# ryought/dbgphmm

Hardware: AMD Instinct MI355X
Metric: read-bases/sec through forward+backward P(R|X) (higher is better)
Workload: dtype f64

## Files before the change

dbgphmm_amd/csrc/api.cpp:

```cpp
#include <chrono>
#include <cstdlib>
#include <cmath>
#include <cstring>

#include "phmm_internal.h"

namespace phmm {

static thread_local std::string g_error;
static thread_local hipStream_t g_stream = nullptr;
static thread_local uint64_t g_ws_limit = 0;
static thread_local CallStats g_stats;
static thread_local bool g_timing = false;

void set_error(const std::string &msg) { g_error = msg; }
int fail(int code, const std::string &msg) {
    g_error = msg;
    return code;
}
hipStream_t current_stream() { return g_stream; }
int &workset_index() {
    static thread_local int idx = 0;
    return idx;
}
ThreadContext capture_thread_context() {
    ThreadContext c{g_ws_limit, g_timing, 0};
    (void)hipGetDevice(&c.device);
    return c;
}
void adopt_thread_context(const ThreadContext &c, hipStream_t stream, int workset) {
    (void)hipSetDevice(c.device);
    g_ws_limit = c.ws_limit;
    g_timing = c.timing;
    g_stream = stream;
    g_stats = CallStats();
    workset_index() = workset;
}
CallStats &stats() { return g_stats; }
bool timing_enabled() { return g_timing; }

uint64_t workspace_limit() {
    if (g_ws_limit) return g_ws_limit;
    size_t fr = 0, tot = 0;
    if (hipMemGetInfo(&fr, &tot) != hipSuccess) return (uint64_t)16 << 30;
    return (uint64_t)(0.8 * (double)fr);
}

static Knobs g_knobs;
const Knobs &knobs() { return g_knobs; }
void refresh_knobs() {
    auto flag = [](const char *n) {
        const char *e = std::getenv(n);
        return e != nullptr && e[0] != '\0' && !(e[0] == '0' && e[1] == '\0');
    };
    auto num = [](const char *n, int dflt) {
        const char *e = std::getenv(n);
        return e ? std::atoi(e) : dflt;
    };
    Knobs k;
    k.trace = flag("PHMM_TRACE");
    k.no_lean = flag("PHMM_NO_LEAN");
    k.no_wide_class = flag("PHMM_NO_WIDE_CLASS");
    k.no_packed = flag("PHMM_NO_PACKED");
    k.packed_cpl = num("PHMM_PACKED_CPL", 0);
    k.no_exact_hinted = flag("PHMM_NO_EXACT_HINTED");
    k.no_exact_dense = flag("PHMM_NO_EXACT_DENSE");
    k.no_wide_hinted = flag("PHMM_NO_WIDE_HINTED");
    k.wide_hinted = flag("PHMM_WIDE_HINTED") && !k.no_wide_hinted;
    k.wide_hinted_cpb = num("PHMM_WIDE_HINTED_CPB", 0);
    if (k.wide_hinted_cpb != 1 && k.wide_hinted_cpb != 2 && k.wide_hinted_cpb != 4) k.wide_hinted_cpb = 0;
    k.no_side_worker = flag("PHMM_NO_SIDE_WORKER");
    k.no_wide_handover = flag("PHMM_NO_WIDE_HANDOVER");
    k.workers = std::max(1, std::min(MAX_WORKERS, num("PHMM_WORKERS", 1)));
    k.warm_cols = num("PHMM_WARM_COLS", 0);
    k.chunk_groups = std::max(0, num("PHMM_CHUNK_GROUPS", 0));
    k.no_keep_all = flag("PHMM_NO_KEEP_ALL");
    k.pipeline_min_groups = std::max(1, num("PHMM_PIPELINE_MIN_GROUPS", 8));
    k.no_runmax = flag("PHMM_NO_RUNMAX");
    k.force_radix = flag("PHMM_FORCE_RADIX");
    k.no_bwd_skip = flag("PHMM_NO_BWD_SKIP");
    k.serial_emit = flag("PHMM_SERIAL_EMIT");
    k.emit_high_priority = flag("PHMM_EMIT_HIGH_PRIORITY");
    k.no_dma = flag("PHMM_NO_DMA");
    k.bwd_dma = flag("PHMM_BWD_DMA");
    k.dense_streams = num("PHMM_DENSE_STREAMS", 0);
    k.dense_w = num("PHMM_DENSE_W", 0);
    k.dense_npt = num("PHMM_DENSE_NPT", 0);
    if (const char *e = std::getenv("PHMM_MEM_FRACTION")) k.mem_fraction = std::min(0.97, std::max(0.1, std::atof(e)));
    g_knobs = k;
}

void trace(const char *tag) {
    if (!g_knobs.trace) return;
    static thread_local std::chrono::steady_clock::time_point last = std::chrono::steady_clock::now();
    (void)hipStreamSynchronize(g_stream);
    const auto now = std::chrono::steady_clock::now();
    static const auto t0 = std::chrono::steady_clock::now();
    std::fprintf(stderr, "[phmm trace] w%d @%9.2f %-28s %8.2f ms\n", workset_index(),
                 std::chrono::duration<double, std::milli>(now - t0).count(), tag,
                 std::chrono::duration<double, std::milli>(now - last).count());
    last = now;
}

uint64_t table_budget(const DevicePool &pool, uint64_t reserve) {
    if (g_ws_limit) return g_ws_limit;
    size_t fr = 0, tot = 0;
    if (hipMemGetInfo(&fr, &tot) != hipSuccess) return (uint64_t)16 << 30;
    const double frac = g_knobs.mem_fraction > 0.0 ? g_knobs.mem_fraction : 0.9;
    const double b = frac * (double)(fr + pool.owned_table_bytes()) - (double)reserve;
    return (uint64_t)std::max(b, 64.0 * 1024 * 1024);
}
uint64_t planned_budget(const DevicePool &pool) {
    if (g_ws_limit) return g_ws_limit;
    size_t fr = 0, tot = 0;
    if (hipMemGetInfo(&fr, &tot) != hipSuccess) return (uint64_t)16 << 30;
    const double frac = g_knobs.mem_fraction > 0.0 ? g_knobs.mem_fraction : 0.95;
    return (uint64_t)(frac * (double)(fr + pool.owned_bytes()));
}

static std::mutex g_pool_mu;
static DevicePool *g_pools[64] = {};
DevicePool &device_pool() {
    int dev = 0;
    (void)hipGetDevice(&dev);
    if (dev < 0 || dev >= 64) PHMM_THROW(PHMM_ENODEVICE, "device index out of range");
    std::lock_guard<std::mutex> lk(g_pool_mu);
    if (!g_pools[dev]) {
        g_pools[dev] = new DevicePool();
        g_pools[dev]->device = dev;
    }
    return *g_pools[dev];
}
void DevicePool::recycle(DevBuf &b) {
    if (!b.p) return;
    std::lock_guard<std::mutex> lk(spare_mu);
    if (b.bytes < ((size_t)1 << 20) || b.bytes > SPARE_BYTES) {
        b.release();
        return;
    }
    while (!spare.empty() && (spare.size() >= SPARE_MAX || spare_total + b.bytes > SPARE_BYTES)) {
        (void)hipFree(spare.front().first);
        spare_total -= spare.front().second;
        spare.erase(spare.begin());
    }
    spare_total += b.bytes;
    const size_t n = b.bytes;
    spare.emplace_back(b.detach(), n);
}
void DevicePool::take(DevBuf &b, size_t n) {
    if (n <= b.bytes) return;
    {
        std::lock_guard<std::mutex> lk(spare_mu);
        int best = -1;
        for (int i = 0; i < (int)spare.size(); i++)
            if (spare[i].second >= n && spare[i].second <= 2 * n &&
                (best < 0 || spare[i].second < spare[best].second))
                best = i;
        if (best >= 0) {
            b.adopt(spare[best].first, spare[best].second);
            spare_total -= spare[best].second;
            spare.erase(spare.begin() + best);
            return;
        }
    }
    b.reserve(n);
}
void DevicePool::flush_spares() {
    std::lock_guard<std::mutex> lk(spare_mu);
    for (auto &e : spare) (void)hipFree(e.first);
    spare.clear();
    spare_total = 0;
}
void flush_spare_buffers() { device_pool().flush_spares(); }

void DevicePool::release() {
    flush_spares();
    for (auto &w : wsets) w.release();
    ws_out.release();
    for (auto &ws : wstream)
        if (ws) {
            (void)hipStreamDestroy(ws);
            ws = nullptr;
        }
    for (auto &ws : cstream)
        if (ws) {
            (void)hipStreamDestroy(ws);
            ws = nullptr;
        }
    for (auto &we : cevent)
        for (auto &e : we)
            if (e) {
                (void)hipEventDestroy(e);
                e = nullptr;
            }
}

void copy_out(void *dst, const void *src_dev, size_t bytes) {
    if (!dst || !bytes) return;
    hipPointerAttribute_t at;
    const bool dev = hipPointerGetAttributes(&at, dst) == hipSuccess && at.type == hipMemoryTypeDevice;
    if (!dev) (void)hipGetLastError();
    HIP_CHECK(hipMemcpyAsync(dst, src_dev, bytes, dev ? hipMemcpyDeviceToDevice : hipMemcpyDeviceToHost,
                             current_stream()));
    HIP_CHECK(hipStreamSynchronize(current_stream()));
}

void put_bytes(void *dst, const void *src, size_t n) {
    if (!dst || !n) return;
    hipPointerAttribute_t at;
    if (hipPointerGetAttributes(&at, dst) == hipSuccess && at.type == hipMemoryTypeDevice) {
        HIP_CHECK(hipMemcpyAsync(dst, src, n, hipMemcpyHostToDevice, current_stream()));
        HIP_CHECK(hipStreamSynchronize(current_stream()));
    } else {
        (void)hipGetLastError();
        std::memcpy(dst, src, n);
    }
}
void put_doubles(double *dst, const double *src, size_t n) { put_bytes(dst, src, n * sizeof(double)); }

void mappings_materialize_host(const phmm_mappings *cmp) {
    if (cmp->host_valid) return;
    auto *mp = const_cast<phmm_mappings *>(cmp);
    mp->pos_off.resize(mp->total_pos + 1);
    mp->nodes.resize(mp->total_entries);
    mp->logp.resize(mp->total_entries);
    HIP_CHECK(hipMemcpy(mp->pos_off.data(), mp->d_pos_off.p, sizeof(uint64_t) * (mp->total_pos + 1), hipMemcpyDeviceToHost));
    if (mp->total_entries) {
        HIP_CHECK(hipMemcpy(mp->nodes.data(), mp->d_nodes.p, sizeof(uint32_t) * mp->total_entries, hipMemcpyDeviceToHost));
        HIP_CHECK(hipMemcpy(mp->logp.data(), mp->d_logp.p, sizeof(double) * mp->total_entries, hipMemcpyDeviceToHost));
    }
    mp->host_valid = true;
}

// ... 758 lines not shown
```

dbgphmm_amd/csrc/dense.hip:

```cpp
#include <algorithm>
#include <cmath>
#include <cstring>
#include <numeric>
#include <type_traits>

#include "dense_internal.h"
#include "lds_dma.h"

#ifndef PHMM_FWD_PF
#define PHMM_FWD_PF 2
#endif
#ifndef PHMM_BWD_PF
#define PHMM_BWD_PF 1
#endif
#ifndef PHMM_SMALLW_WAVES
#define PHMM_SMALLW_WAVES 3
#endif

namespace phmm {


__device__ __forceinline__ int xcd_block(int b, int nblk8) {
    int per = nblk8 >> 3;
    return (b & 7) * per + (b >> 3);
}

__device__ __forceinline__ NodeRec load_node(const NodeRec *nodes, int k) {
    typedef const NodeRec __attribute__((address_space(4))) *KPtr;
    const KPtr q = (KPtr)(uintptr_t)nodes;
    NodeRec r;
    r.init = q[k].init;
    r.dinit = q[k].dinit;
    r.tdinit = q[k].tdinit;
    r.emis = q[k].emis;
    r.flags = q[k].flags;
    return r;
}

__device__ __forceinline__ void wait_vmcnt(int n) {
#define PHMM_VMW(k) case k: asm volatile("s_waitcnt vmcnt(" #k ")" ::: "memory"); break;
    switch (n) {
        PHMM_VMW(1) PHMM_VMW(2) PHMM_VMW(3) PHMM_VMW(4) PHMM_VMW(5) PHMM_VMW(6) PHMM_VMW(7) PHMM_VMW(8)
        PHMM_VMW(9) PHMM_VMW(10) PHMM_VMW(11) PHMM_VMW(12) PHMM_VMW(13) PHMM_VMW(14) PHMM_VMW(15) PHMM_VMW(16)
        PHMM_VMW(17) PHMM_VMW(18) PHMM_VMW(19) PHMM_VMW(20) PHMM_VMW(21) PHMM_VMW(22) PHMM_VMW(23) PHMM_VMW(24)
        PHMM_VMW(25) PHMM_VMW(26) PHMM_VMW(27) PHMM_VMW(28) PHMM_VMW(29) PHMM_VMW(30) PHMM_VMW(31)
    default: asm volatile("s_waitcnt vmcnt(0)" ::: "memory"); break;
    }
#undef PHMM_VMW
}
#ifndef PHMM_DMA_DEPTH
#define PHMM_DMA_DEPTH 4
#endif
static constexpr int DMA_DEPTH = PHMM_DMA_DEPTH;
static_assert(DMA_DEPTH - 1 + DMA_DEPTH * 3 <= 31, "vmcnt immediates");

__device__ __forceinline__ int exp_of_bits(unsigned long long bits) {
    int be = (int)((bits >> 52) & 0x7ff);
    if (bits == 0ull) return 0;
    if (be == 0) return -1022;
    return be - 1022;
}
__device__ __forceinline__ double pow2(int e) {
    return __longlong_as_double((long long)(e + 1023) << 52);
}

template <int W, class Op>
__device__ __forceinline__ double block_reduce_rows(double v, Op op, double *lds) {
#pragma unroll
    for (int off = W; off < 64; off <<= 1) v = op(v, __shfl_xor(v, off));
    const int wave = threadIdx.x >> 6, lane = threadIdx.x & 63;
    __syncthreads();
    if (lane < W) lds[wave * 64 + lane] = v;
    __syncthreads();
    double out = v;
    if (threadIdx.x < W) {
        out = lds[threadIdx.x];
#pragma unroll
        for (int w = 1; w < BLOCK / 64; w++) out = op(out, lds[w * 64 + threadIdx.x]);
    }
    return out;
}
template <int W> __device__ __forceinline__ double lanes_sum(double v) {
    if (W == 16) {
        auto ror = [](double x, auto ctrl) {
            const long long b = __double_as_longlong(x);
            const int lo = __builtin_amdgcn_update_dpp(0, (int)(b & 0xffffffffll), decltype(ctrl)::value, 0xf, 0xf, false);
            const int hi = __builtin_amdgcn_update_dpp(0, (int)(b >> 32), decltype(ctrl)::value, 0xf, 0xf, false);
            return __longlong_as_double(((long long)hi << 32) | (long long)(unsigned int)lo);
        };
        v += ror(v, std::integral_constant<int, 0x128>());
        v += ror(v, std::integral_constant<int, 0x124>());
        v += ror(v, std::integral_constant<int, 0x122>());
        v += ror(v, std::integral_constant<int, 0x121>());
        return v;
    }
#pragma unroll
    for (int off = 1; off < W; off <<= 1) v += __shfl_xor(v, off);
    return v;
}

struct OpMax {
    __device__ double operator()(double a, double b) const { return a > b ? a : b; }
};
struct OpAdd {
    __device__ double operator()(double a, double b) const { return a + b; }
};

template <int W, bool DMA>
__global__ void __launch_bounds__(BLOCK, (W == 64 ? 4 : PHMM_SMALLW_WAVES)) fwd_step(const DenseArgs a, const int pos) {
    __shared__ double lds[(BLOCK / 64) * 64];
    constexpr bool DMA_ = DMA && W == 64;
    __shared__ double ring[DMA_ ? (BLOCK / 64) * DMA_DEPTH * 128 : 1];
    const int g = blockIdx.y + a.g_off;
    const int lb = xcd_block(blockIdx.x, a.nblk8);
    constexpr int ROWS = BLOCK / W;
    const int r = threadIdx.x % W;
    const int row = threadIdx.x / W;
    const int len = a.len[g * W + r];
    const bool active = a.wf_sw == nullptr || a.wf_sw[g * W + r] < 0;
    const bool newcol = active && pos < len;
    const bool have_prev = active && pos >= 1 && pos <= len;
    const bool fin = have_prev && pos == len;
    if (!__syncthreads_or(newcol || have_prev)) return;
    const LinParams &lp = a.lp;
    const size_t NW = (size_t)a.N * W;

    int Epos = 0;
    double sc = 1.0, isc = 1.0, ibs = 0.0;
    double thrL = INFINITY, thrU = INFINITY;
    bool collect = false;
    if (have_prev) {
        const unsigned long long cm = a.cmaxF[((size_t)g * a.Lc + (pos - 1)) * W + r];
        const int Eprev = a.FE[((size_t)g * (a.Lc + 1) + (pos - 1)) * W + r];
        const double ib_st = exp(a.logib[pos - 1] - (double)Eprev * LN2);
        const unsigned long long ibb = (unsigned long long)__double_as_longlong(ib_st);
        const int e = exp_of_bits(cm > ibb ? cm : ibb);
        sc = pow2(-e);
        isc = pow2(e);
        Epos = Eprev + e;
        ibs = exp(a.logib[pos - 1] - (double)Epos * LN2);
        if (a.wf_sw) {
            const double cmF = __longlong_as_double((long long)cm) * sc;
            thrL = cmF * a.wf_ratio;
            thrU = (a.wf_ub_a * cmF + a.wf_ub_b * lp.p_ID * ibs) * (1.0 + 1e-9) * a.wf_ratio;
            collect = a.wf_mode[g * W + r] != 0;
        }
    }
    const uint8_t x = newcol ? a.bases[((size_t)g * a.Lc + pos) * W + r] : (uint8_t)0;

    const double *pm = a.Fm + ((size_t)g * a.Lc + (pos > 0 ? pos - 1 : 0)) * NW;
    const double *pi = a.Fi + ((size_t)g * a.Lc + (pos > 0 ? pos - 1 : 0)) * NW;
    double *pd = a.Fd + ((size_t)g * a.Lc + (pos > 0 ? pos - 1 : 0)) * NW;
// ... 101 lines not shown
                        D4 = wg[0] + q * (wg[1] + q * (wg[2] + q * wg[3]));
                        D5 = wg[0] + q * (wg[1] + q * (wg[2] + q * (wg[3] + q * wg[4])));
                        Tk = 0.0;
#pragma unroll
                        for (int h = H - 1; h >= 1; h--)
                            if (h <= lp.n_max_gaps + 1) Tk = wg[h] + q * Tk;
                        nvalid = 1;
                    }
                    m1 = wm0;
                    i1 = wi0;
                    const int G = lp.n_max_gaps;
                    dacc = G == 4 ? D5 : (G == 3 ? D4 : (G == 2 ? D3 : (G == 1 ? D2 : D1)));
                    tacc = Tk;
                } else {
                    m1 = i1 = dacc = tacc = 0.0;
                    const uint32_t o0 = a.fc_off[k], o1 = a.fc_off[k + 1];
                    for (uint32_t q = o0; q < o1; q++) {
                        const FwdEntry en = a.fc[q];
                        const size_t ix = (size_t)en.node * W + r;
                        const double vm = pm[ix] * sc, vi = pi[ix] * sc;
                        const double gg = lp.p_MD * vm + lp.p_ID * vi;
                        m1 += en.w1 * vm;
                        i1 += en.w1 * vi;
                        dacc += en.wD * gg;
                        tacc += en.wT * gg;
                    }
                }
                const double dprev = dacc + c * nr.dinit;
                const double td = tacc + c * nr.tdinit;
                if (have_prev) pd[ik] = dprev * isc;
                mnew = pe * (lp.p_MM * m1 + lp.p_IM * i1 + lp.p_DM * td + nr.init * cb);
                inew = lp.p_random * (lp.p_MI * om + lp.p_II * oi + lp.p_DI * dprev);
                const double tk = om + oi + dprev;
                if (want_e) esum += tk;
                if (have_prev) tmax = fmax(tmax, tk);
                if (tk > thrL) {
                    nsub += tk > thrU ? 1 : 0;
                    if (collect) {
                        const int gi = g * W + r;
                        const int slot = atomicAdd(&a.wf_cnt[gi], 1);
                        if (slot < WF_CAP) {
                            a.wf_node[(size_t)gi * WF_CAP + slot] = (uint32_t)k;
                            a.wf_tot[(size_t)gi * WF_CAP + slot] = tk * isc;
                        }
                    }
                }
                {
                    const double gk = lp.p_MD * om + lp.p_ID * oi, q = lp.p_DD;
                    Tk = dacc;
                    D5 = gk + q * D4;
                    D4 = gk + q * D3;
                    D3 = gk + q * D2;
                    D2 = gk + q * D1;
                    D1 = gk;
                }
                wm0 = om;
                wi0 = oi;
            }
            if (newcol) {
                cm_[ik] = mnew;
                ci_[ik] = inew;
                vmax = fmax(vmax, fmax(mnew, inew));
            }
          }
        }
    }
    if (DMA_) asm volatile("s_waitcnt vmcnt(0)" ::: "memory");
    const double bm = block_reduce_rows<W>(vmax, OpMax(), lds);
    if (threadIdx.x < W && newcol && lb < a.nblk)
        atomicMax(&a.cmaxF[((size_t)g * a.Lc + pos) * W + r], (unsigned long long)__double_as_longlong(bm));
    if (a.tmaxF && pos >= 1) {
        const double bt = block_reduce_rows<W>(tmax * isc, OpMax(), lds);
        if (threadIdx.x < W && have_prev && lb < a.nblk)
            atomicMax(&a.tmaxF[((size_t)g * a.Lc + (pos - 1)) * W + r], (unsigned long long)__double_as_longlong(bt));
    }
    if (a.wf_sw) {
        const double bn = block_reduce_rows<W>((double)nsub, OpAdd(), lds);
        if (threadIdx.x < W && bn > 0.0) atomicAdd(&a.wf_sub[g * W + r], (int)bn);
    }
    if (a.eall || __syncthreads_or(fin)) {
        const double bs = block_reduce_rows<W>(esum, OpAdd(), lds);
        if (threadIdx.x < W && want_e && lb < a.nblk) {
            const size_t col = a.eall ? (size_t)(pos - 1) : 0;
            const size_t ecols = a.eall ? (size_t)a.Lc : 1;
            a.epart[(((size_t)g * ecols + col) * a.nblk8 + lb) * W + r] = bs;
        }
    }
    if (lb == 0 && threadIdx.x < W && (newcol || have_prev))
        a.FE[((size_t)g * (a.Lc + 1) + pos) * W + r] = Epos;
}

template <int W>
__global__ void __launch_bounds__(BLOCK) fwd_init(const DenseArgs a) {
    __shared__ double lds[(BLOCK / 64) * 64];
    const int g = blockIdx.y + a.g_off;
    const int lb = xcd_block(blockIdx.x, a.nblk8);
    constexpr int ROWS = BLOCK / W;
    const int r = threadIdx.x % W, row = threadIdx.x / W;
    const int len = a.len[g * W + r];
    const bool active = a.wf_sw == nullptr || a.wf_sw[g * W + r] < 0;
    const bool newcol = active && 0 < len;
    if (!__syncthreads_or(newcol)) return;
    const size_t NW = (size_t)a.N * W;
    double *cm_ = a.Fm + (size_t)g * a.Lc * NW, *ci_ = a.Fi + (size_t)g * a.Lc * NW;
    const uint8_t x = newcol ? a.bases[(size_t)g * a.Lc * W + r] : (uint8_t)0;
    double vmax = 0.0;
    if (lb < a.nblk && newcol) {
        const int kbase = lb * (a.npt * ROWS) + row * a.npt;
        for (int j = 0; j < a.npt; j++) {
            const int k = kbase + j;
            if (k >= a.N) break;
            const NodeRec nr = a.nodes[k];
            const double mnew = ((uint8_t)nr.emis == x ? a.lp.p_match : a.lp.p_mismatch) * nr.init * a.lp.p_MM;
            cm_[(size_t)k * W + r] = mnew;
            ci_[(size_t)k * W + r] = 0.0;
            vmax = fmax(vmax, mnew);
        }
    }
    const double bm = block_reduce_rows<W>(vmax, OpMax(), lds);
    if (threadIdx.x < W && newcol && lb < a.nblk)
        atomicMax(&a.cmaxF[(size_t)g * a.Lc * W + r], (unsigned long long)__double_as_longlong(bm));
    if (lb == 0 && threadIdx.x < W && newcol) a.FE[(size_t)g * (a.Lc + 1) * W + r] = 0;
}

template <int W>
__global__ void __launch_bounds__(BLOCK) fwd_finish(const DenseArgs a) {
    __shared__ double lds[(BLOCK / 64) * 64];
    const int g = blockIdx.x;
    const int col = blockIdx.y;
    constexpr int ROWS = BLOCK / W;
    const int r = threadIdx.x % W, row = threadIdx.x / W;
    const int len = a.len[g * W + r];
    const size_t ecols = a.eall ? (size_t)a.Lc : 1;
    double s = 0.0;
    const bool live = a.eall ? col < len : len > 0;
    if (live)
        for (int b = row; b < a.nblk; b += ROWS)
            s += a.epart[(((size_t)g * ecols + col) * a.nblk8 + b) * W + r];
    const double tot = block_reduce_rows<W>(s, OpAdd(), lds);
    if (threadIdx.x < W && live) {
        const int E = a.FE[((size_t)g * (a.Lc + 1) + (a.eall ? col + 1 : len)) * W + r];
        const double lp = log(a.lp.p_end * tot) + (double)E * LN2;
        if (a.eall) a.logE[((size_t)g * a.Lc + col) * W + r] = lp;
        if (!a.eall || col == len - 1) a.logPf[g * W + r] = lp;
    }
}

__device__ __forceinline__ double dev_logadd(double x, double y) {
    const double hi = x >= y ? x : y, lo = x >= y ? y : x;
    if (lo == -INFINITY) return hi;
    return hi + log1p(exp(lo - hi));
}

template <int W>
__device__ __forceinline__ void bwd_chain(const DenseArgs &a, int g, int p, double *lds) {
    constexpr int ROWS = BLOCK / W;
    const int r = threadIdx.x % W, row = threadIdx.x / W;
    const int len = a.len[g * W + r];
    const bool live = p < len && (!a.bstart || p <= (a.bstart[g * W + r] & ~(1 << 30)));
    double s1 = 0.0, s2 = 0.0;
    if (live) {
        const double *bp = a.bpart + ((size_t)(p & 1) * a.ng + g) * a.nblk8 * W * 2;
        for (int b = row; b < a.nblk; b += ROWS) {
            s1 += bp[((size_t)b * W + r) * 2 + 0];
            s2 += bp[((size_t)b * W + r) * 2 + 1];
        }
    }
    const double t1 = block_reduce_rows<W>(s1, OpAdd(), lds);
    const double t2 = block_reduce_rows<W>(s2, OpAdd(), lds);
    if (threadIdx.x < W && live) {
        const size_t ix = ((size_t)g * (a.Lc + 1) + p) * W + r;
        const double E = (double)a.BE[ix] * LN2;
        const double ibn = (p + 1 < len) ? a.logibB[ix + W] : -INFINITY;
        const double lr = log(a.lp.p_random);
        a.logmbB[ix] = dev_logadd(log(t1) + E, log(a.lp.p_MI) + lr + ibn);
        a.logibB[ix] = dev_logadd(log(t2) + E, log(a.lp.p_II) + lr + ibn);
    }
}

static constexpr int BDMA_DEPTH = 3;
static constexpr int BDMA_SLOT = 5 * 64;
template <int W, bool DMA>
__global__ void __launch_bounds__(BLOCK, (W == 64 ? 4 : PHMM_SMALLW_WAVES)) bwd_step(const DenseArgs a, const int pos) {
    __shared__ double lds[(BLOCK / 64) * 64];
    constexpr bool DMA_ = DMA && W == 64;
    __shared__ double ring[DMA_ ? (BLOCK / 64) * BDMA_DEPTH * BDMA_SLOT : 1];
    const int g = blockIdx.y + a.g_off;
    const int lb = xcd_block(blockIdx.x, a.nblk8);
    constexpr int ROWS = BLOCK / W;
    const int r = threadIdx.x % W;
    const int row = threadIdx.x / W;
    const int len = a.len[g * W + r];
    const int braw = a.bstart ? a.bstart[g * W + r] : len - 1;
    const bool sparse_tail = (braw & (1 << 30)) != 0;
    const int bstart = braw & ~(1 << 30);
    const bool live = pos < len && pos <= bstart;
    const bool first = live && pos == len - 1;
    const LinParams &lp = a.lp;
    const size_t NW = (size_t)a.N * W;

    if (lb == 0 && pos + 1 < a.Lc) bwd_chain<W>(a, g, pos + 1, lds);

    bool compute = true;
    int hull_first = 0, hull_top = a.npt - 1;
    if (W == 64 && a.skA) {
        compute = false;
        const int rho = __builtin_amdgcn_readfirstlane(lb * ROWS + row);
        if (__any(live) && rho < a.nrun) {
            const size_t gs = (size_t)g * a.nseg, gr = (size_t)g * a.nrun, par = (size_t)a.ng * a.nrun;
            const uint32_t *hh = a.skH + gs;
            const uint8_t *an = a.skA + (size_t)((pos + 1) & 1) * par + gr;
            const int sh = pos + 1 < 31 ? pos + 1 : 31;
            const int sprs = segs_per_run_log2(a.npt), spr = 1 << sprs;
            const unsigned anyfirst = __any(first) ? 1u : 0u;
            const int ls = threadIdx.x & 63;
            const int sg = rho * spr + ls;
            unsigned f = 0;
            if (ls < spr && sg < a.nseg) {
                f = (hh[sg] >> sh) | (((unsigned)an[rho] >> ls) & 1u) | anyfirst;
                const uint32_t o0 = a.rs_off[sg], o1 = a.rs_off[sg + 1];
                for (uint32_t q = o0; q < o1 && !f; q++) {
                    const uint32_t t = a.rs[q];
                    f = (hh[t] >> sh) | (((unsigned)an[t >> sprs] >> (t & (uint32_t)(spr - 1))) & 1u);
                }
            }
            const unsigned mask = (unsigned)__builtin_amdgcn_readfirstlane((int)(unsigned)__ballot(f != 0));
            const int kb = rho * a.npt;
            compute = seg_hull(mask, a.sseg, a.npt - 1 < a.N - 1 - kb ? a.npt - 1 : a.N - 1 - kb, &hull_first, &hull_top);
            if (ls == 0) a.skA[(size_t)(pos & 1) * par + gr + rho] = (uint8_t)mask;
        }
    }
    if (!__syncthreads_or(live && (compute || lb == 0))) {
        if (threadIdx.x < W && lb < a.nblk) {
            double *bp = a.bpart + ((size_t)(pos & 1) * a.ng + g) * a.nblk8 * W * 2;
            bp[((size_t)lb * W + r) * 2 + 0] = 0.0;
            bp[((size_t)lb * W + r) * 2 + 1] = 0.0;
        }
        if (a.want_map && a.Prun) a.Prun[((size_t)g * a.nblk8 + lb) * BLOCK + threadIdx.x] = 0.0;
        return;
    }

    int Epos = 0;
    double sc = 1.0;
    if (live && !first) {
        const unsigned long long cm = a.cmaxB[((size_t)g * a.Lc + (pos + 1)) * W + r];
        const int e = exp_of_bits(cm);
        sc = pow2(-e);
        Epos = a.BE[((size_t)g * (a.Lc + 1) + (pos + 1)) * W + r] + e;
    }
    const uint8_t x = live ? a.bases[((size_t)g * a.Lc + pos) * W + r] : (uint8_t)0;
    const int cn = a.bcols == 2 ? ((pos + 1) & 1) : (pos + 1 < a.Lc ? pos + 1 : 0);
    const int cc = a.bcols == 2 ? (pos & 1) : pos;
    const double *nm = a.Bm + ((size_t)g * a.bcols + cn) * NW;
    const double *ni = a.Bi + ((size_t)g * a.bcols + cn) * NW;
    double *om = a.Bm + ((size_t)g * a.bcols + cc) * NW;
    double *oi = a.Bi + ((size_t)g * a.bcols + cc) * NW;
    double *od = a.Bd ? a.Bd + ((size_t)g * a.bcols + cc) * NW : nullptr;

    double wgt = 0.0, wgt2 = 0.0;
    const double *fm = nullptr, *fi = nullptr, *fd = nullptr, *gm = nullptr, *gi = nullptr, *gd = nullptr;
    const bool want_post = a.want_freq || a.want_map;
    if (want_post && live) {
        const double lpf = a.logPf[g * W + r];
        if (lpf > -INFINITY) {
            if (pos >= 1) {
                const int fe = a.FE[((size_t)g * (a.Lc + 1) + (pos - 1)) * W + r];
                wgt = exp((double)(fe + Epos) * LN2 - lpf);
            }
            if (first && !sparse_tail) {
                const int fe = a.FE[((size_t)g * (a.Lc + 1) + pos) * W + r];
                wgt2 = exp((double)fe * LN2 - lpf) * lp.p_end;
            }
        }
    }
    if (want_post) {
        const size_t cprev = ((size_t)g * a.Lc + (pos > 0 ? pos - 1 : 0)) * NW;
        const size_t ccur = ((size_t)g * a.Lc + pos) * NW;
        fm = a.Fm + cprev; fi = a.Fi + cprev; fd = a.Fd + cprev;
        gm = a.Fm + ccur; gi = a.Fi + ccur; gd = a.Fd + ccur;
    }

    double vmax = 0.0, s1 = 0.0, s2 = 0.0, pmx = 0.0, pmx2 = 0.0;
    double *Pa = a.want_map ? a.Pa + (size_t)g * NW : nullptr;
    double *Pb = a.want_map ? a.Pb + (size_t)g * NW : nullptr;
    if (lb < a.nblk && compute) {
        constexpr int H = CHAIN_HOPS;
        const int kbase = lb * (a.npt * ROWS) + row * a.npt + hull_first;
        double E1 = 0.0, E2 = 0.0, E3 = 0.0, E4 = 0.0, E5 = 0.0, Q1 = 0.0, Q2 = 0.0, Q3 = 0.0, Q4 = 0.0, Q5 = 0.0, TE = 0.0;
        int nvalid = 0;
        constexpr int PFB = DMA_ ? BDMA_DEPTH : PHMM_BWD_PF;
        double nx_m[PFB], nx_i[PFB], nx_fm[PFB], nx_fi[PFB], nx_fd[PFB];
        const double *lfm = want_post ? fm : nm, *lfi = want_post ? fi : nm, *lfd = want_post ? fd : nm;
        const int jtop = hull_top < a.N - 1 - kbase ? hull_top : a.N - 1 - kbase;
        const int l64 = threadIdx.x & 63;
        const double *srcA = (l64 < 32 ? nm : ni) + 2 * (l64 & 31);
        const double *srcB = (l64 < 32 ? lfm : lfi) + 2 * (l64 & 31);
        const double *srcC = lfd + 2 * (l64 & 31);
        const uint32_t ring_base =
            DMA_ ? (uint32_t)__builtin_amdgcn_readfirstlane(
                       (int)(uint32_t)(uintptr_t)&ring[(threadIdx.x >> 6) * BDMA_DEPTH * BDMA_SLOT])
                 : 0u;
        const double *ring_w = &ring[DMA_ ? (threadIdx.x >> 6) * BDMA_DEPTH * BDMA_SLOT : 0];
        const int n1 = __any(live) ? 2 + (od ? 1 : 0) : 0;
        if (W == 64 && a.skcells) {
            const unsigned long long nlive = (unsigned long long)__popcll(__ballot(live));
            if (l64 == 0 && jtop >= 0) atomicAdd(a.skcells, nlive * (unsigned long long)(jtop + 1));
        }
        const int ns = n1 + ((a.want_map && __any(live)) ? 1 : 0) + (a.want_freq ? 2 : 0);
#pragma unroll
        for (int u = 0; u < PFB; u++) {
            int v0 = kbase + (jtop - u > 0 ? jtop - u : 0);
            if (v0 > a.N - 1) v0 = a.N - 1;
            if (W == 64) v0 = __builtin_amdgcn_readfirstlane(v0);
            const size_t i0 = (size_t)(live ? v0 : 0) * W + r;
            nx_m[u] = nx_i[u] = nx_fm[u] = nx_fi[u] = nx_fd[u] = 0.0;
            if (DMA_) {
                const uint32_t slot = ring_base + (uint32_t)u * (BDMA_SLOT * 8);
                glds16(srcA + (size_t)v0 * W, slot);
                glds16(srcB + (size_t)v0 * W, slot + 1024u);
                if (l64 < 32) glds16(srcC + (size_t)v0 * W, slot + 2048u);
            } else if (jtop >= 0) {
                nx_m[u] = nm[i0];
                nx_i[u] = ni[i0];
                nx_fm[u] = lfm[i0];
                nx_fi[u] = lfi[i0];
                nx_fd[u] = lfd[i0];
            }
        }
        NodeRec nr_next{};
        if (jtop >= 0) {
            int v0 = kbase + jtop;
            if (W == 64) v0 = __builtin_amdgcn_readfirstlane(v0);
            nr_next = load_node(a.nodes, v0);
        }
        for (int j0 = jtop; j0 >= 0; j0 -= PFB) {
#pragma unroll
          for (int u = 0; u < PFB; u++) {
            const int j = j0 - u;
            if (j < 0) continue;
            int v = kbase + j;
            if (W == 64) v = __builtin_amdgcn_readfirstlane(v);
            double contrib = 0.0;
            {
                const NodeRec nr = nr_next;
                const size_t iv = (size_t)v * W + r;
                const bool first_group = j0 == jtop;
                double cur_m, cur_i;
                if (DMA_) {
                    wait_vmcnt(2 + 3 * (PFB - 1) + (first_group ? u : PFB) * ns);
                    cur_m = ring_w[u * BDMA_SLOT + r] * sc;
                    cur_i = ring_w[u * BDMA_SLOT + 64 + r] * sc;
                } else {
                    cur_m = nx_m[u] * sc;
                    cur_i = nx_i[u] * sc;
                }
                if (W == 64) {
                    asm volatile("" : : "s"(nr.flags), "s"(nr.emis), "v"(cur_m), "v"(cur_i));
                    __builtin_amdgcn_sched_barrier(0);
                }
                int vp = v - PFB > kbase ? v - PFB : kbase;
                if (W == 64) vp = __builtin_amdgcn_readfirstlane(vp);
                {
                    int vn = v - 1 > kbase ? v - 1 : kbase;
                    if (W == 64) vn = __builtin_amdgcn_readfirstlane(vn);
                    nr_next = load_node(a.nodes, vn);
                    if (DMA_) {
                        glds16(srcA + (size_t)vp * W, ring_base + (uint32_t)u * (BDMA_SLOT * 8));
                    } else {
                        nx_m[u] = nm[(size_t)(live ? vp : 0) * W + r];
                        nx_i[u] = ni[(size_t)(live ? vp : 0) * W + r];
                    }
                }
                double cur_fm = nx_fm[u], cur_fi = nx_fi[u], cur_fd = nx_fd[u];
                const double m0 = first ? lp.p_end : cur_m;
                const double q0 = lp.p_random * (first ? lp.p_end : cur_i);
                const double ev = (uint8_t)nr.emis == x ? lp.p_match : lp.p_mismatch;
                double a1, ad, at, qd, qt;
                if (a.hop_mode) {
                    if (!((nr.flags & CHAIN_B) && nvalid)) {
                        double wh[H], wq[H];
#pragma unroll
                        for (int h = 0; h < H; h++) wh[h] = wq[h] = 0.0;
                        const uint32_t o0 = a.bh_off[v], o1 = a.bh_off[v + 1];
                        for (uint32_t q = o0; q < o1; q++) {
                            const HopEntry en = a.bh[q];
                            const size_t ix = (size_t)en.node * W + r;
                            const double mu = first ? lp.p_end : nm[ix] * sc;
                            const double iu = first ? lp.p_end : ni[ix] * sc;
                            const double hv = en.w * ((uint8_t)(en.hop_emis >> 8) == x ? lp.p_match : lp.p_mismatch) * mu;
                            const double qv = en.w * lp.p_random * iu;
                            const int hh = (int)(en.hop_emis & 0xff) - 1;
#pragma unroll
                            for (int h = 0; h < H; h++)
                                if (hh == h) {
                                    wh[h] += hv;
                                    wq[h] += qv;
                                }
                        }
                        const double q = lp.p_DD;
                        E1 = wh[0];
                        E2 = wh[0] + q * wh[1];
                        E3 = wh[0] + q * (wh[1] + q * wh[2]);
                        E4 = wh[0] + q * (wh[1] + q * (wh[2] + q * wh[3]));
                        E5 = wh[0] + q * (wh[1] + q * (wh[2] + q * (wh[3] + q * wh[4])));
                        Q1 = wq[0];
                        Q2 = wq[0] + q * wq[1];
                        Q3 = wq[0] + q * (wq[1] + q * wq[2]);
                        Q4 = wq[0] + q * (wq[1] + q * (wq[2] + q * wq[3]));
                        Q5 = wq[0] + q * (wq[1] + q * (wq[2] + q * (wq[3] + q * wq[4])));
                        TE = 0.0;
#pragma unroll
                        for (int h = H - 1; h >= 1; h--)
                            if (h <= lp.n_max_gaps + 1) TE = wh[h] + q * TE;
                        nvalid = 1;
                    }
                    const int G = lp.n_max_gaps;
                    a1 = E1;
                    ad = G == 4 ? E5 : (G == 3 ? E4 : (G == 2 ? E3 : (G == 1 ? E2 : E1)));
                    at = TE;
                    qt = G == 4 ? Q5 : (G == 3 ? Q4 : (G == 2 ? Q3 : (G == 1 ? Q2 : Q1)));
                    qd = lp.p_DD * (G == 4 ? Q4 : (G == 3 ? Q3 : (G == 2 ? Q2 : (G == 1 ? Q1 : 0.0))));
                } else {
                    a1 = ad = at = qd = qt = 0.0;
                    const uint32_t o0 = a.bc_off[v], o1 = a.bc_off[v + 1];
                    for (uint32_t q = o0; q < o1; q++) {
                        const BwdEntry en = a.bc[q];
                        const size_t ix = (size_t)en.node * W + r;
                        const double mu = first ? lp.p_end : nm[ix] * sc;
                        const double iu = first ? lp.p_end : ni[ix] * sc;
                        const double h = ((uint8_t)en.emis == x ? lp.p_match : lp.p_mismatch) * mu;
                        const double qq = lp.p_random * iu;
                        a1 += en.c1 * h;
                        ad += en.cAd * h;
                        at += en.cAt * h;
                        qd += en.cQd * qq;
                        qt += en.cAd * qq;
                    }
                }
                if (a.hop_mode) {
                    const double hk = ev * m0, q = lp.p_DD;
                    TE = ad;
                    E5 = hk + q * E4;
                    E4 = hk + q * E3;
                    E3 = hk + q * E2;
                    E2 = hk + q * E1;
                    E1 = hk;
                    Q5 = q0 + q * Q4;
                    Q4 = q0 + q * Q3;
                    Q3 = q0 + q * Q2;
                    Q2 = q0 + q * Q1;
                    Q1 = q0;
                }
                const double d = lp.p_DM * ad + lp.p_DI * (q0 + qd);
                const double td = lp.p_DM * at + lp.p_DI * qt;
                const double m = lp.p_MM * a1 + lp.p_MD * td + lp.p_MI * q0;
                const double i = lp.p_IM * a1 + lp.p_ID * td + lp.p_II * q0;
                if (live) {
                    om[iv] = m;
                    oi[iv] = i;
                    if (od) od[iv] = d;
                    vmax = fmax(vmax, fmax(m, i));
                    const double in = nr.init;
                    s1 += in * (lp.p_MM * ev * m0 + lp.p_MD * d);
                    s2 += in * (lp.p_IM * ev * m0 + lp.p_ID * d);
                }
                if (DMA_) {
                    wait_vmcnt(1 + n1 + 3 * (PFB - 1) + (first_group ? (u < PFB - 1 ? u : PFB - 1) : PFB - 1) * ns);
                    cur_fm = ring_w[u * BDMA_SLOT + 128 + r];
                    cur_fi = ring_w[u * BDMA_SLOT + 192 + r];
                    cur_fd = ring_w[u * BDMA_SLOT + 256 + r];
                }
                double c1 = 0.0, c2 = 0.0;
                if (wgt != 0.0) c1 = wgt * (cur_fm * m + cur_fi * i + cur_fd * d);
                if (wgt2 != 0.0) c2 = wgt2 * (gm[iv] + gi[iv] + gd[iv]);
                contrib = c1 + c2;
                if (a.want_map && live) {
                    Pa[iv] = c1;
                    pmx = fmax(pmx, c1);
                    if (first && !sparse_tail) {
                        Pb[iv] = c2;
                        pmx2 = fmax(pmx2, c2);
                    }
                }
                {
                    if (DMA_) {
                        if (W == 64) {
                            asm volatile("" : : "v"(contrib));
                            __builtin_amdgcn_sched_barrier(0);
                        }
                        const uint32_t slot = ring_base + (uint32_t)u * (BDMA_SLOT * 8);
                        glds16(srcB + (size_t)vp * W, slot + 1024u);
                        if (l64 < 32) glds16(srcC + (size_t)vp * W, slot + 2048u);
                    } else {
                        nx_fm[u] = lfm[(size_t)(live ? vp : 0) * W + r];
                        nx_fi[u] = lfi[(size_t)(live ? vp : 0) * W + r];
                        nx_fd[u] = lfd[(size_t)(live ? vp : 0) * W + r];
                    }
                }
            }
            if (a.want_freq) {
                const double tot = lanes_sum<W>(contrib);
                if (r == 0) (void)unsafeAtomicAdd(&a.accg[(size_t)g * a.N + v], tot);
            }
          }
        }
    }
    if (DMA_) asm volatile("s_waitcnt vmcnt(0)" ::: "memory");
    const double bmx = block_reduce_rows<W>(vmax, OpMax(), lds);
    if (threadIdx.x < W && live && lb < a.nblk)
        atomicMax(&a.cmaxB[((size_t)g * a.Lc + pos) * W + r], (unsigned long long)__double_as_longlong(bmx));
    if (a.want_map) {
        if (a.Prun) a.Prun[((size_t)g * a.nblk8 + lb) * BLOCK + threadIdx.x] = pmx;
        const double p1 = block_reduce_rows<W>(pmx, OpMax(), lds);
        if (threadIdx.x < W && live && lb < a.nblk)
            atomicMax(&a.pmax[((size_t)g * (a.Lc + 1) + pos) * W + r], (unsigned long long)__double_as_longlong(p1));
        const double p2 = block_reduce_rows<W>(pmx2, OpMax(), lds);
        if (threadIdx.x < W && first && !sparse_tail && lb < a.nblk)
            atomicMax(&a.pmax[((size_t)g * (a.Lc + 1) + len) * W + r], (unsigned long long)__double_as_longlong(p2));
    }
    const double t1 = block_reduce_rows<W>(s1, OpAdd(), lds);
    const double t2 = block_reduce_rows<W>(s2, OpAdd(), lds);
    if (threadIdx.x < W && lb < a.nblk) {
        double *bp = a.bpart + ((size_t)(pos & 1) * a.ng + g) * a.nblk8 * W * 2;
        bp[((size_t)lb * W + r) * 2 + 0] = t1;
        bp[((size_t)lb * W + r) * 2 + 1] = t2;
    }
    if (lb == 0 && threadIdx.x < W && live) a.BE[((size_t)g * (a.Lc + 1) + pos) * W + r] = Epos;
}

template <int W>
__global__ void __launch_bounds__(BLOCK) bwd_finish(const DenseArgs a) {
    __shared__ double lds[(BLOCK / 64) * 64];
    bwd_chain<W>(a, blockIdx.x, 0, lds);
}

__global__ void __launch_bounds__(BLOCK) freq_reduce(const double *accg, int ng, int N, double *out, int accumulate) {
    const int k = blockIdx.x * BLOCK + threadIdx.x;
    if (k >= N) return;
    double s = accumulate ? out[k] : 0.0;
    for (int g = 0; g < ng; g++) s += accg[(size_t)g * N + k];
    out[k] = s;
}

template <int W>
__global__ void __launch_bounds__(BLOCK) edge_freq_kernel(const DenseArgs a, const uint32_t *esrc, const uint32_t *edst,
                                                          const double *trans, const double *init, int E, double *accE,
                                                          double *accI) {
    constexpr int ROWS = BLOCK / W;
    const int g = blockIdx.y;
    const int r = threadIdx.x % W, row = threadIdx.x / W;
    const int item = blockIdx.x * ROWS + row;
    if (item >= E + a.N) return;
    const bool is_edge = item < E;
    const int k = is_edge ? (int)esrc[item] : 0;
    const int l = is_edge ? (int)edst[item] : item - E;
    const double t = is_edge ? trans[item] : init[l];
    const int len = a.len[g * W + r];
    const LinParams &lp = a.lp;
    const size_t NW = (size_t)a.N * W;
    const double lpf = a.logPf[g * W + r];
    const uint8_t el = a.emis[l];
    double acc = 0.0;
    if (len > 0 && lpf > -INFINITY && t != 0.0) {
        const int *FE = a.FE + (size_t)g * (a.Lc + 1) * W + r;
        const int *BE = a.BE + (size_t)g * (a.Lc + 1) * W + r;
        for (int i = is_edge ? 1 : 0; i <= len; i++) {
            double sm, sd;
            int fe = 0;
            double lib = 0.0;
            if (is_edge) {
                const size_t ix = ((size_t)g * a.Lc + (i - 1)) * NW + (size_t)k * W + r;
                const double fm = a.Fm[ix], fi = a.Fi[ix], fd = a.Fd[ix];
                sm = lp.p_MM * fm + lp.p_IM * fi + lp.p_DM * fd;
                sd = lp.p_MD * fm + lp.p_ID * fi + lp.p_DD * fd;
                fe = FE[(size_t)(i - 1) * W];
            } else if (i == 0) {
                sm = lp.p_MM;
                sd = lp.p_MD;
            } else {
                sm = lp.p_IM;
                sd = lp.p_ID;
                lib = a.logib[i - 1];
            }
            double term = 0.0;
            if (i < len) {
                const uint8_t x = a.bases[((size_t)g * a.Lc + i) * W + r];
                const double pe = el == x ? lp.p_match : lp.p_mismatch;
                double bm;
                int be;
                if (i + 1 < len) {
                    bm = a.Bm[((size_t)g * a.bcols + (i + 1)) * NW + (size_t)l * W + r];
                    be = BE[(size_t)(i + 1) * W];
                } else {
                    bm = lp.p_end;
                    be = 0;
                }
                const double v1 = sm * pe * bm;
                if (v1 != 0.0) term += v1 * exp(lib + (double)(fe + be) * LN2 - lpf);
                const double bd = a.Bd[((size_t)g * a.bcols + i) * NW + (size_t)l * W + r];
                const double v2 = sd * bd;
                if (v2 != 0.0) term += v2 * exp(lib + (double)(fe + BE[(size_t)i * W]) * LN2 - lpf);
            } else {
                const double v3 = sd * lp.p_end;
                if (v3 != 0.0) term += v3 * exp(lib + (double)fe * LN2 - lpf);
            }
            acc += t * term;
        }
    }
    const double tot = lanes_sum<W>(acc);
    if (r == 0) {
        if (is_edge) accE[(size_t)g * E + item] = tot;
        else accI[(size_t)g * a.N + l] = tot;
    }
}

__global__ void __launch_bounds__(BLOCK) to_log_tables(const double *T, const int *E, int Lc, int N, int L,
                                                       double *out) {
    const size_t idx = (size_t)blockIdx.x * BLOCK + threadIdx.x;
    if (idx >= (size_t)L * N) return;
    const int pos = (int)(idx / N);
    const double v = T[idx];
    out[idx] = v >= 2.2250738585072014e-308 ? log(v) + (double)E[pos] * LN2 : -INFINITY;
}


struct Timer {
    hipEvent_t a = nullptr, b = nullptr;
    bool on;
    explicit Timer(bool on_) : on(on_) {
        if (on) {
            HIP_CHECK(hipEventCreate(&a));
            HIP_CHECK(hipEventCreate(&b));
        }
    }
    ~Timer() {
        if (a) (void)hipEventDestroy(a);
        if (b) (void)hipEventDestroy(b);
    }
    void start() {
        if (on) HIP_CHECK(hipEventRecord(a, current_stream()));
    }
    double stop() {
        if (!on) return 0.0;
        HIP_CHECK(hipEventRecord(b, current_stream()));
        HIP_CHECK(hipEventSynchronize(b));
        float ms = 0;
        HIP_CHECK(hipEventElapsedTime(&ms, a, b));
        return ms;
    }
};

template <int W> static void launch_fwd_one(const DenseArgs &a0, int pos, int g_off = 0, int g_cnt = -1, hipStream_t s = nullptr) {
    const bool dma = !knobs().no_dma;
    DenseArgs a = a0;
    a.g_off = g_off;
    if (g_cnt < 0) {
        g_cnt = a.ng;
        s = current_stream();
    }
    if (pos == 0) hipLaunchKernelGGL(fwd_init<W>, dim3(a.nblk8, g_cnt), dim3(BLOCK), 0, s, a);
    else if (W == 64 && dma && a.npt % DMA_DEPTH == 0)
        hipLaunchKernelGGL((fwd_step<W, true>), dim3(a.nblk8, g_cnt), dim3(BLOCK), 0, s, a, pos);
    else
        hipLaunchKernelGGL((fwd_step<W, false>), dim3(a.nblk8, g_cnt), dim3(BLOCK), 0, s, a, pos);
}
template <int W> static void launch_bwd_one(const DenseArgs &a0, int pos, int g_off = 0, int g_cnt = -1, hipStream_t s = nullptr) {
    const bool dma = knobs().bwd_dma;
    DenseArgs a = a0;
    a.g_off = g_off;
    if (g_cnt < 0) {
        g_cnt = a.ng;
        s = current_stream();
    }
    if (W == 64 && dma)
        hipLaunchKernelGGL((bwd_step<W, true>), dim3(a.nblk8, g_cnt), dim3(BLOCK), 0, s, a, pos);
    else
        hipLaunchKernelGGL((bwd_step<W, false>), dim3(a.nblk8, g_cnt), dim3(BLOCK), 0, s, a, pos);
}
static int dense_stream_count(const DenseArgs &a) {
    const int forced = knobs().dense_streams;
    int k = forced;
    if (k <= 0) {
        const long blocks = (long)a.nblk8 * a.ng;
        k = blocks >= 4096 ? 1 : (blocks >= 1536 ? 2 : 3);
    }
    return std::max(1, std::min(std::min(k, MAX_WORKERS), a.ng));
}
template <int W>
void launch_chunk(phmm_model *m, const DenseArgs &a, bool do_bwd, CallStats &st, bool timing) {
    hipStream_t s = current_stream();
    dim3 blk(BLOCK);
    Timer tf(timing), tb(timing);
    const int K = dense_stream_count(a);
    hipStream_t ks[MAX_WORKERS] = {s, nullptr, nullptr, nullptr};
    hipEvent_t fork = nullptr, join[MAX_WORKERS] = {};
    if (K > 1) {
        HIP_CHECK(hipEventCreateWithFlags(&fork, hipEventDisableTiming));
        for (int k = 1; k < K; k++) {
            if (!m->pool->wstream[k]) HIP_CHECK(hipStreamCreateWithFlags(&m->pool->wstream[k], hipStreamNonBlocking));
            ks[k] = m->pool->wstream[k];
            HIP_CHECK(hipEventCreateWithFlags(&join[k], hipEventDisableTiming));
        }
    }
    auto g_lo = [&](int k) { return (int)((long)a.ng * k / K); };
    auto fan_out = [&] {
        if (K == 1) return;
        HIP_CHECK(hipEventRecord(fork, s));
        for (int k = 1; k < K; k++) HIP_CHECK(hipStreamWaitEvent(ks[k], fork, 0));
    };
    auto fan_in = [&] {
        for (int k = 1; k < K; k++) {
            HIP_CHECK(hipEventRecord(join[k], ks[k]));
            HIP_CHECK(hipStreamWaitEvent(s, join[k], 0));
        }
    };
    tf.start();
    fan_out();
    for (int pos = 0; pos <= a.Lc; pos++)
        for (int k = 0; k < K; k++) launch_fwd_one<W>(a, pos, g_lo(k), g_lo(k + 1) - g_lo(k), ks[k]);
    fan_in();
    st.ms[0] += tf.stop();
    st.launches[0] += (uint64_t)a.Lc + 1;
    hipLaunchKernelGGL(fwd_finish<W>, dim3(a.ng, a.eall ? a.Lc : 1), blk, 0, s, a);
    if (do_bwd) {
        tb.start();
        fan_out();
        for (int pos = a.Lc - 1; pos >= 0; pos--)
            for (int k = 0; k < K; k++) launch_bwd_one<W>(a, pos, g_lo(k), g_lo(k + 1) - g_lo(k), ks[k]);
        fan_in();
        st.ms[1] += tb.stop();
        st.launches[1] += (uint64_t)a.Lc;
        hipLaunchKernelGGL(bwd_finish<W>, dim3(a.ng), blk, 0, s, a);
    }
    const hipError_t le = hipGetLastError();
    if (fork) (void)hipEventDestroy(fork);
    for (int k = 1; k < K; k++)
        if (join[k]) (void)hipEventDestroy(join[k]);
    HIP_CHECK(le);
}

template <int W> static void launch_fwd_fin(const DenseArgs &a) {
    hipLaunchKernelGGL(fwd_finish<W>, dim3(a.ng, a.eall ? a.Lc : 1), dim3(BLOCK), 0, current_stream(), a);
}
#define PHMM_W_SWITCH(W, CALL)                                  \
    switch (W) {                                                \
    case 1: CALL(1); break;                                     \
    case 2: CALL(2); break;                                     \
    case 4: CALL(4); break;                                     \
    case 8: CALL(8); break;                                     \
    case 16: CALL(16); break;                                   \
    case 32: CALL(32); break;                                   \
    case 64: CALL(64); break;                                   \
    default: PHMM_THROW(PHMM_EINTERNAL, "bad read-group width"); \
    }
void launch_fwd_step(int W, const DenseArgs &a, int pos) {
#define CALL_(w) launch_fwd_one<w>(a, pos)
    PHMM_W_SWITCH(W, CALL_)
#undef CALL_
}
void launch_bwd_step(int W, const DenseArgs &a, int pos) {
#define CALL_(w) launch_bwd_one<w>(a, pos)
    PHMM_W_SWITCH(W, CALL_)
#undef CALL_
}
template <int W> static void launch_bwd_fin(const DenseArgs &a) {
    hipLaunchKernelGGL(bwd_finish<W>, dim3(a.ng), dim3(BLOCK), 0, current_stream(), a);
}
void launch_bwd_finish(int W, const DenseArgs &a) {
#define CALL_(w) launch_bwd_fin<w>(a)
    PHMM_W_SWITCH(W, CALL_)
#undef CALL_
    HIP_CHECK(hipGetLastError());
}
void launch_fwd_finish(int W, const DenseArgs &a) {
#define CALL_(w) launch_fwd_fin<w>(a)
    PHMM_W_SWITCH(W, CALL_)
#undef CALL_
}

void launch_chunk_w(phmm_model *m, int W, const DenseArgs &a, bool do_bwd, CallStats &st, bool timing) {
    switch (W) {
    case 1: launch_chunk<1>(m, a, do_bwd, st, timing); break;
    case 2: launch_chunk<2>(m, a, do_bwd, st, timing); break;
    case 4: launch_chunk<4>(m, a, do_bwd, st, timing); break;
    case 8: launch_chunk<8>(m, a, do_bwd, st, timing); break;
    case 16: launch_chunk<16>(m, a, do_bwd, st, timing); break;
    case 32: launch_chunk<32>(m, a, do_bwd, st, timing); break;
    case 64: launch_chunk<64>(m, a, do_bwd, st, timing); break;
    default: PHMM_THROW(PHMM_EINTERNAL, "bad read-group width");
    }
}

int choose_width(uint64_t R) {
    if (R <= 64) {
        int W = 1;
        while ((uint64_t)W < R && W < 32) W <<= 1;
        return W;
    }
    for (int W = 64; W >= 2; W >>= 1) {
        uint64_t padded = (R + W - 1) / W * W;
        if ((padded - R) * 16 <= padded) return W;
    }
    return 1;
}

size_t align_up(size_t v, size_t a) { return (v + a - 1) / a * a; }

struct Carver {
    char *base;
    size_t off = 0;
    explicit Carver(void *b) : base((char *)b) {}
    template <class T> T *take(size_t n) {
        off = align_up(off, 256);
        T *p = base ? (T *)(base + off) : nullptr;
        off += n * sizeof(T);
        return p;
    }
};

Plan make_plan(const phmm_model *m, const phmm_reads *reads, int forced_w) {
    std::vector<uint32_t> all(reads->R);
    std::iota(all.begin(), all.end(), 0u);
    Plan p = make_plan_ids(m, reads, all);
    if (forced_w > 0 && forced_w != p.W) {
        p.W = forced_w;
        p.ng_total = (int)((p.order.size() + p.W - 1) / p.W);
        const int rows = BLOCK / p.W;
        p.nblk = (int)((m->N + (int64_t)p.npt * rows - 1) / ((int64_t)p.npt * rows));
        p.nblk8 = (p.nblk + 7) / 8 * 8;
    }
    return p;
}

Plan make_plan_ids(const phmm_model *m, const phmm_reads *reads, const std::vector<uint32_t> &ids) {
    Plan p;
    const uint64_t R = ids.size();
    const int forced_w = 0;
    p.order = ids;
    std::stable_sort(p.order.begin(), p.order.end(), [&](uint32_t x, uint32_t y) {
        return reads->off[x + 1] - reads->off[x] > reads->off[y + 1] - reads->off[y];
    });
    p.W = forced_w > 0 ? forced_w : choose_width(R);
    {
        const int w = knobs().dense_w;
        if (w == 1 || w == 2 || w == 4 || w == 8 || w == 16 || w == 32 || w == 64) p.W = w;
    }
    p.ng_total = (int)((R + p.W - 1) / p.W);
    const int rows = BLOCK / p.W;
    int npt = 8;
    const double lanes_total = (double)m->N * (double)(p.ng_total * p.W);
    while (npt < 64 && lanes_total / (npt * 2) >= 524288.0) npt *= 2;
    while ((int64_t)((m->N + (int64_t)npt * rows - 1) / ((int64_t)npt * rows)) > 4096 && npt < 64) npt *= 2;
    if (knobs().dense_npt > 0) npt = std::max(2, std::min(256, knobs().dense_npt & ~1));
    p.npt = npt;
    p.nblk = (int)((m->N + (int64_t)npt * rows - 1) / ((int64_t)npt * rows));
    p.nblk8 = (p.nblk + 7) / 8 * 8;
    return p;
}

void layout(DenseArgs &a, int W, bool full_b, void *tables, void *misc, size_t &tb, size_t &mb, bool backward_only) {
    const size_t NW = (size_t)a.N * W;
    Carver t(tables), s(misc);
    const size_t fcols = backward_only ? 0 : (size_t)a.Lc;
    a.Fm = t.take<double>((size_t)a.ng * fcols * NW);
    a.Fi = t.take<double>((size_t)a.ng * fcols * NW);
    a.Fd = t.take<double>((size_t)a.ng * fcols * NW);
    a.bcols = full_b ? a.Lc : 2;
    a.Bm = t.take<double>((size_t)a.ng * a.bcols * NW);
    a.Bi = t.take<double>((size_t)a.ng * a.bcols * NW);
    a.Bd = (full_b || backward_only) ? t.take<double>((size_t)a.ng * a.bcols * NW) : nullptr;
    tb = t.off;
    a.bases = s.take<uint8_t>((size_t)a.ng * a.Lc * W);
    a.len = s.take<int>((size_t)a.ng * W);
    a.FE = s.take<int>((size_t)a.ng * (a.Lc + 1) * W);
    a.BE = s.take<int>((size_t)a.ng * (a.Lc + 1) * W);
    a.cmaxF = s.take<unsigned long long>((size_t)a.ng * a.Lc * W);
    a.cmaxB = s.take<unsigned long long>((size_t)a.ng * a.Lc * W);
    a.epart = s.take<double>((size_t)a.ng * (a.eall ? a.Lc : 1) * a.nblk8 * W);
    a.logPf = s.take<double>((size_t)a.ng * W);
    a.logE = s.take<double>(a.eall ? (size_t)a.ng * a.Lc * W : 1);
    a.bpart = s.take<double>((size_t)2 * a.ng * a.nblk8 * W * 2);
    a.logmbB = s.take<double>((size_t)a.ng * (a.Lc + 1) * W);
    a.logibB = s.take<double>((size_t)a.ng * (a.Lc + 1) * W);
    a.accg = s.take<double>((size_t)a.ng * a.N);
    a.logib = s.take<double>((size_t)a.Lc + 1);
    a.tmaxF = s.take<unsigned long long>((size_t)a.ng * a.Lc * W);
    a.pmax = s.take<unsigned long long>((size_t)a.ng * (a.Lc + 1) * W);
    mb = s.off;
}

void fill_model_args(DenseArgs &a, const phmm_model *m) {
    const ModelDev &d = m->dev;
    a.N = (int)m->N;
    a.nodes = d.nodes.as<NodeRec>();
    a.emis = d.emis.as<uint8_t>();
    a.init = d.init.as<double>();
    a.dinit = d.dinit.as<double>();
    a.tdinit = d.tdinit.as<double>();
    a.fc_off = d.fc_off.as<uint32_t>();
    a.fc = d.fc_ent.as<FwdEntry>();
    a.bc_off = d.bc_off.as<uint32_t>();
    a.bc = d.bc_ent.as<BwdEntry>();
    a.lp = m->lin;
    a.fh_off = d.fh_off.as<uint32_t>();
    a.fh = d.fh_ent.as<HopEntry>();
    a.bh_off = d.bh_off.as<uint32_t>();
    a.bh = d.bh_ent.as<HopEntry>();
    a.hop_mode = m->lin.n_max_gaps + 2 <= CHAIN_HOPS ? 1 : 0;
}

void host_logib(const phmm_model *m, size_t n, std::vector<double> &out) {
    out.resize(n + 1);
    const phmm_params &p = m->params;
    double ib = p.p_random + p.p_MI;
    for (size_t i = 0; i <= n; i++) {
        out[i] = ib;
        ib = p.p_random + p.p_II + ib;
    }
}
// ... 350 lines not shown
```

dbgphmm_amd/csrc/dense_internal.h:

```cpp
#pragma once

#include <vector>

#include "phmm_internal.h"
#include "seg_hull.h"

namespace phmm {

static constexpr double LN2 = 0.693147180559945309417232121458;
static constexpr int BLOCK = 256;

struct DenseArgs {
    int N, ng, Lc, nblk, npt;
    int g_off;
    const NodeRec *nodes;
    const uint8_t *emis;
    const double *init, *dinit, *tdinit;
    const uint32_t *fc_off;
    const FwdEntry *fc;
    const uint32_t *bc_off;
    const BwdEntry *bc;
    const uint32_t *fh_off, *bh_off;
    const HopEntry *fh, *bh;
    int hop_mode;
    LinParams lp;
    const double *logib;
    const uint8_t *bases;
    const int *len;
    double *Fm, *Fi, *Fd;
    int *FE;
    unsigned long long *cmaxF;
    double *epart;
    int eall;
    double *logPf;
    double *logE;
    double *Bm, *Bi, *Bd;
    int bcols;
    int *BE;
    unsigned long long *cmaxB;
    double *bpart;
    double *logmbB, *logibB;
    double *accg;
    int want_freq;
    int nblk8;
    unsigned long long *tmaxF;
    const int *bstart;
    int want_map;
    double *Pa, *Pb;
    double *Prun;
    unsigned long long *pmax;
    const int *wf_sw;
    const uint8_t *wf_mode;
    int *wf_sub;
    int *wf_cnt;
    uint32_t *wf_node;
    double *wf_tot;
    double wf_ratio;
    double wf_ub_a, wf_ub_b;
    const uint32_t *rs_off = nullptr, *rs = nullptr;
    uint32_t *skH = nullptr;
    uint8_t *skA = nullptr;
    int nrun = 0, nseg = 0, sseg = 1;
    unsigned long long *skcells = nullptr;
};
static constexpr int WF_CAP = 1024;


struct Plan {
    int W, ng_total, npt, nblk, nblk8;
    std::vector<uint32_t> order;
};

Plan make_plan(const phmm_model *m, const phmm_reads *reads, int forced_w);
Plan make_plan_ids(const phmm_model *m, const phmm_reads *reads, const std::vector<uint32_t> &ids);
void layout(DenseArgs &a, int W, bool full_b, void *tables, void *misc, size_t &tb, size_t &mb,
            bool backward_only = false);
void fill_model_args(DenseArgs &a, const phmm_model *m);
void host_logib(const phmm_model *m, size_t n, std::vector<double> &out);
void launch_fwd_step(int W, const DenseArgs &a, int pos);
void launch_fwd_finish(int W, const DenseArgs &a);
void launch_bwd_step(int W, const DenseArgs &a, int pos);
void launch_bwd_finish(int W, const DenseArgs &a);

struct ExactTables {
    double *f_m, *f_i, *f_d, *f_scal, *b_m, *b_i, *b_d, *b_scal;
};
void exact_dense_reads(phmm_model *m, const uint8_t *bases, const uint64_t *off, const std::vector<uint32_t> &ids, double *lf,
                       double *lb, double *freq_dev, const ExactTables *tabs, double *edge_freq_dev = nullptr,
                       double *init_freq_dev = nullptr);
bool certify_dense(int N, int len, double log2P, const int *FE, const double *log2maxF, const int *BE, const double *log2maxB,
                   double log2_p_end);
bool certify_dense_cells(int N, int len, const int *E, const double *log2max, bool backward);

}
```

dbgphmm_amd/csrc/mapping_flow.hip:

```cpp
#include <algorithm>
#include <cmath>
#include <cstring>
#include <memory>

#include <hipcub/hipcub.hpp>

#include "sparse_dyn.h"
#include "lean_bwd_kernel.h"
#include "wide_bwd_kernel.h"

namespace phmm {

static constexpr int KMAX = PHMM_MAX_ACTIVE_NODES;

template <int CAP> struct FRec {
    double m[CAP], i[CAP], d[CAP];
    uint32_t id[CAP];
    int n, na, E;
};

template <int CAP> __device__ bool load_record(const RecPool &p, uint64_t pos_index, FRec<CAP> &f) {
    const uint64_t o1 = p.off[pos_index];
    if (o1 == 0) return false;
    const uint8_t *rec = p.base + (o1 - 8);
// ... 320 lines not shown
        }
        wave_sync();
        if (!emit_mapping<CAP>(a.mpool, q0 + (uint64_t)(pos - 1), fr.id, val, fr.n, a.ratio_lin, true, order, a.topk))
            err |= SP_ERR_POOL;
        if (!a.list_off && a.max_steps > 0 && !err && ++steps_done >= a.max_steps && cur.n <= 64 && pos - 1 >= s0 + 1) {
            stopped = true;
            stop_at = pos - 1;
            break;
        }
    }
    if (a.list_off) {
        if (stopped) err |= SP_ERR_CAPACITY;
        if (lane == 0) a.stop[gi] = stopped ? stop_at : s0;
        if (a.logb && lane == 0 && have_cols && !stopped && !err)
            a.logb[gi] = log(mb) + (double)cols[0].E * SP_LN2;
    } else if (stopped && !err) {
        if (have_cols && stop_at < len) {
            const Col<CAP> &c = cols[(stop_at + 1) & 1];
            BHandoff &h = a.hand[gi];
            if (c.n > HANDOFF_CAP) err |= SP_ERR_CAPACITY;
            else {
                if (lane == 0) {
                    h.n = c.n;
                    h.E = c.E;
                    h.ib = ib;
                }
                for (int j = lane; j < c.n; j += 64) {
                    h.id[j] = c.id[j];
                    h.m[j] = c.m[j];
                    h.i[j] = c.i[j];
                    h.d[j] = c.d[j];
                }
            }
        }
        if (lane == 0) a.stop[gi] = stop_at;
    } else if (!err) {
        if (have_cols) {
            const Col<CAP> &c = cols[(s0 + 1) & 1];
            const size_t NW = (size_t)a.d.N * a.W;
            const int pc = (s0 + 1) & 1;
            double *bm = a.d.Bm + ((size_t)g * a.d.bcols + pc) * NW;
            double *bi = a.d.Bi + ((size_t)g * a.d.bcols + pc) * NW;
            double mx = 0.0;
            for (int j = lane; j < c.n; j += 64) {
                bm[(size_t)c.id[j] * a.W + r] = c.m[j];
                bi[(size_t)c.id[j] * a.W + r] = c.i[j];
                if (a.d.skH && (c.m[j] != 0.0 || c.i[j] != 0.0))
                    atomicOr(&a.d.skH[(size_t)g * a.d.nseg + c.id[j] / (uint32_t)a.d.sseg], 1u << (s0 + 1 < 31 ? s0 + 1 : 31));
                mx = fmax(mx, fmax(c.m[j], c.i[j]));
            }
            mx = wave_max(mx);
            if (lane == 0) {
                a.d.cmaxB[((size_t)g * a.d.Lc + (s0 + 1)) * a.W + r] = (unsigned long long)__double_as_longlong(mx);
                a.d.BE[((size_t)g * (a.d.Lc + 1) + (s0 + 1)) * a.W + r] = c.E;
                a.d.logibB[((size_t)g * (a.d.Lc + 1) + (s0 + 1)) * a.W + r] = log(ib) + (double)c.E * SP_LN2;
            }
        }
        if (lane == 0) a.stop[gi] = s0;
    }
    for (int off = 32; off >= 1; off >>= 1) err |= (uint32_t)__shfl_xor((int)err, off);
    if (lane == 0) a.err[gi] = err;
}

struct DenseMapArgs {
    DenseArgs d;
    int W;
    RecPool mpool;
    const uint64_t *lane_pos0;
    int *cntA, *cntB;
    uint32_t *candA_node, *candB_node;
    double *candA_val, *candB_val;
    double ratio_lin;
    int topk;
    uint32_t *err;
    unsigned long long *eoff;
    int force_radix;
    uint32_t *wl_small;
    uint32_t *wl_big;
    int *wl_count;
};

template <int W>
__global__ void __launch_bounds__(BLOCK) post_collect(const DenseMapArgs ma, const int pos) {
    const DenseArgs &a = ma.d;
    const int g = blockIdx.y, lb = blockIdx.x;
    constexpr int ROWS = BLOCK / W;
    const int r = threadIdx.x % W, row = threadIdx.x / W;
    const int gi = g * W + r;
    const int len = a.len[gi];
    const int braw = a.bstart[gi];
    const bool sparse_tail = (braw & (1 << 30)) != 0;
    const int bstart = braw & ~(1 << 30);
    const bool live = pos < len && pos <= bstart;
    const bool doA = live && pos >= 1;
    const bool doB = live && pos == len - 1 && !sparse_tail;
    if (lb >= a.nblk) return;
    const size_t NW = (size_t)a.N * W;
    if (a.Prun && doA) {
        const double thr = __longlong_as_double((long long)a.pmax[((size_t)g * (a.Lc + 1) + pos) * W + r]) * ma.ratio_lin;
        const double rm = a.Prun[((size_t)g * a.nblk8 + lb) * BLOCK + threadIdx.x];
        if (rm > 0.0 && rm > thr) {
            const double *P = a.Pa + (size_t)g * NW;
            const int k0 = lb * (a.npt * ROWS) + row * a.npt;
            uint32_t *cn = ma.candA_node + (size_t)gi * KMAX;
            double *cv = ma.candA_val + (size_t)gi * KMAX;
            int local = 0;
            for (int j = 0; j < a.npt && k0 + j < a.N; j++) {
                const double t = P[(size_t)(k0 + j) * W + r];
                local += (t > 0.0 && t > thr) ? 1 : 0;
            }
            int slot = atomicAdd(&ma.cntA[gi], local);
            for (int j = 0; j < a.npt && k0 + j < a.N && slot < KMAX; j++) {
                const double t = P[(size_t)(k0 + j) * W + r];
                if (t > 0.0 && t > thr) {
                    cn[slot] = (uint32_t)(k0 + j);
                    cv[slot] = t;
                    slot++;
                }
            }
        }
    }
    const int kbase = lb * (a.npt * ROWS) + row;
    for (int which = (a.Prun ? 1 : 0); which < 2; which++) {
        if (!(which == 0 ? doA : doB)) continue;
        const double *P = (which == 0 ? a.Pa : a.Pb) + (size_t)g * NW;
        const int mi = which == 0 ? pos : len;
        const double thr =
            __longlong_as_double((long long)a.pmax[((size_t)g * (a.Lc + 1) + mi) * W + r]) * ma.ratio_lin;
        int *cnt = which == 0 ? ma.cntA : ma.cntB;
        uint32_t *cn = (which == 0 ? ma.candA_node : ma.candB_node) + (size_t)gi * KMAX;
        double *cv = (which == 0 ? ma.candA_val : ma.candB_val) + (size_t)gi * KMAX;
        int local = 0;
        for (int j = 0; j < a.npt; j++) {
            const int k = kbase + j * ROWS;
            if (k >= a.N) break;
            const double t = P[(size_t)k * W + r];
            local += (t > 0.0 && t > thr) ? 1 : 0;
        }
        if (local == 0) continue;
        int slot = atomicAdd(&cnt[gi], local);
        for (int j = 0; j < a.npt && slot < KMAX; j++) {
            const int k = kbase + j * ROWS;
            if (k >= a.N) break;
            const double t = P[(size_t)k * W + r];
            if (t > 0.0 && t > thr) {
                cn[slot] = (uint32_t)k;
                cv[slot] = t;
                slot++;
            }
        }
    }
}

__device__ int block_top_radix(const double *col, int stride, int N, double thr, uint32_t *ids, double *val) {
    __shared__ unsigned int hist[256];
    __shared__ unsigned long long s_prefix;
    __shared__ int s_k, s_wcnt[BLOCK / 64], s_n;
    const int tid = threadIdx.x, lane = tid & 63, wave = tid >> 6;
    if (tid == 0) {
        s_prefix = 0ull;
        s_k = KMAX;
    }
    __syncthreads();
    for (int shift = 56; shift >= 0; shift -= 8) {
        hist[tid] = 0u;
        __syncthreads();
        const unsigned long long prefix = s_prefix;
        for (int k = tid; k < N; k += BLOCK) {
            const double v = col[(size_t)k * stride];
            if (!(v > thr)) continue;
            const unsigned long long b = (unsigned long long)__double_as_longlong(v);
            if (shift < 56 && (b >> (shift + 8)) != (prefix >> (shift + 8))) continue;
            atomicAdd(&hist[(b >> shift) & 255ull], 1u);
        }
        __syncthreads();
        if (tid == 0) {
            int k = s_k, d = 255;
            for (; d > 0; d--) {
                if ((int)hist[d] >= k) break;
                k -= (int)hist[d];
            }
            s_k = k;
            s_prefix = prefix | ((unsigned long long)d << shift);
        }
        __syncthreads();
    }
    const unsigned long long T = s_prefix;
    if (tid == 0) s_n = 0;
    __syncthreads();
    for (int pass = 0; pass < 2; pass++)
        for (int base = 0; base < N; base += BLOCK) {
            const int k = base + tid;
            double v = 0.0;
            bool take = false;
            if (k < N) {
                v = col[(size_t)k * stride];
                const unsigned long long b = (unsigned long long)__double_as_longlong(v);
                take = v > thr && (pass == 0 ? b > T : b == T);
            }
            const unsigned long long mk = __ballot(take);
            if (lane == 0) s_wcnt[wave] = __popcll(mk);
            __syncthreads();
            int p = s_n + __popcll(mk & ((1ull << lane) - 1ull));
            for (int w = 0; w < wave; w++) p += s_wcnt[w];
            if (take && p < KMAX) {
                ids[p] = (uint32_t)k;
                val[p] = v;
            }
            __syncthreads();
            if (tid == 0) {
                int t = s_n;
                for (int w = 0; w < BLOCK / 64; w++) t += s_wcnt[w];
                s_n = t;
            }
            __syncthreads();
            if (s_n >= KMAX) break;
        }
    __syncthreads();
    return s_n < KMAX ? s_n : KMAX;
}

__global__ void __launch_bounds__(1024) emit_offsets(const DenseMapArgs ma, const int pos, const int lanes) {
    __shared__ unsigned long long part[1024];
    __shared__ unsigned long long s_base;
    const DenseArgs &a = ma.d;
    const int tid = threadIdx.x;
    const int items = 2 * lanes;
    const int per = (items + 1023) / 1024;
    auto bytes_of = [&](int it) -> unsigned long long {
        if (it >= items) return 0ull;
        const int which = it / lanes, gi = it % lanes;
        const int len = a.len[gi];
        if (len == 0) return 0ull;
        const int braw = a.bstart[gi];
        const bool sparse_tail = (braw & (1 << 30)) != 0;
        const int bstart = braw & ~(1 << 30);
        const bool live = pos < len && pos <= bstart;
        const bool mine = which == 0 ? (live && pos >= 1) : (live && pos == len - 1 && !sparse_tail);
        if (!mine) return 0ull;
        const int c = (which == 0 ? ma.cntA : ma.cntB)[gi];
        int k = c < KMAX ? c : KMAX;
        if (ma.topk > 0) {
            const int want = ma.topk < a.N ? ma.topk : a.N;
            k = k > want ? k : want;
        }
        return 8ull + (unsigned long long)((k + 1) & ~1) * 4ull + (unsigned long long)k * 8ull;
    };
    unsigned long long loc = 0ull;
    for (int q = 0; q < per; q++) loc += bytes_of(tid * per + q);
    part[tid] = loc;
    __syncthreads();
    for (int off = 1; off < 1024; off <<= 1) {
        const unsigned long long v = tid >= off ? part[tid - off] : 0ull;
        __syncthreads();
        part[tid] += v;
        __syncthreads();
    }
    if (tid == 1023) s_base = atomicAdd(ma.mpool.top, part[1023]);
    __syncthreads();
    unsigned long long o = s_base + part[tid] - loc;
    for (int q = 0; q < per; q++) {
        const int it = tid * per + q;
        if (it < items) ma.eoff[it] = o;
        o += bytes_of(it);
    }
    auto class_of = [&](int it) -> int {
        if (bytes_of(it) == 0ull) return 0;
        const int c = (it / lanes == 0 ? ma.cntA : ma.cntB)[it % lanes];
        return (ma.topk <= 0 && c >= 1 && c <= 64) ? 1 : 2;
    };
    __syncthreads();
    unsigned long long cl = 0ull;
    for (int q = 0; q < per; q++) {
        const int c = class_of(tid * per + q);
        cl += c == 1 ? 1ull : (c == 2 ? (1ull << 32) : 0ull);
    }
    part[tid] = cl;
    __syncthreads();
    for (int off = 1; off < 1024; off <<= 1) {
        const unsigned long long v = tid >= off ? part[tid - off] : 0ull;
        __syncthreads();
        part[tid] += v;
        __syncthreads();
    }
    unsigned long long at = part[tid] - cl;
    for (int q = 0; q < per; q++) {
        const int it = tid * per + q;
        const int c = class_of(it);
        if (c == 1) ma.wl_small[(uint32_t)at] = (uint32_t)it, at += 1ull;
        else if (c == 2) ma.wl_big[(uint32_t)(at >> 32)] = (uint32_t)it, at += 1ull << 32;
    }
    if (tid == 1023) {
        ma.wl_count[0] = (int)(uint32_t)part[1023];
        ma.wl_count[1] = (int)(uint32_t)(part[1023] >> 32);
    }
}

__global__ void __launch_bounds__(BLOCK) emit_dense_small(const DenseMapArgs ma, const int pos, const int lanes) {
    const DenseArgs &a = ma.d;
    const int wave = threadIdx.x >> 6, lane = threadIdx.x & 63;
    const int n_items = ma.wl_count[0];
    for (int w = blockIdx.x * (BLOCK / 64) + wave; w < n_items; w += gridDim.x * (BLOCK / 64)) {
        const uint32_t it = ma.wl_small[w];
        const int which = (int)(it / (uint32_t)lanes), gi = (int)(it % (uint32_t)lanes);
        int *cnt = which == 0 ? ma.cntA : ma.cntB;
        const int c = cnt[gi];
// ... 109 lines not shown
            if (lane == 0) {
                if (mk) wb = atomicAdd(&s_n, __popcll(mk));
                if (me) wbb = atomicAdd(&s_nb, __popcll(me));
            }
            wb = __shfl(wb, 0);
            wbb = __shfl(wbb, 0);
            const int p = wb + __popcll(mk & ((1ull << lane) - 1ull)), pb = wbb + __popcll(me & ((1ull << lane) - 1ull));
            if (take && p < KMAX) {
                ids[p] = (uint32_t)k;
                val[p] = v;
            }
            if (edge && pb < TOPH_STAGE) {
                bid[pb] = (uint32_t)k;
                bval[pb] = v;
            }
        }
    }
    __syncthreads();
    const int nabove = s_n, nb = s_nb, need = s_need;
    if (nb > TOPH_STAGE) return block_top_radix(col, stride, N, thr, ids, val);
    __syncthreads();
    for (int j = tid; j < nb; j += BLOCK) {
        const double v = bval[j];
        const uint32_t id = bid[j];
        int rank = 0;
        for (int q = 0; q < nb; q++) {
            const double u = bval[q];
            rank += (u > v) || (u == v && bid[q] < id);
        }
        if (rank < need && nabove + rank < KMAX) {
            ids[nabove + rank] = id;
            val[nabove + rank] = v;
        }
    }
    __syncthreads();
    const int tot = nabove + (nb < need ? nb : need);
    return tot < KMAX ? tot : KMAX;
}

__global__ void __launch_bounds__(BLOCK) emit_dense_map(const DenseMapArgs ma, const int pos, const int lanes) {
    __shared__ uint32_t ids[KMAX];
    __shared__ double val[KMAX];
    __shared__ uint16_t order[KMAX];
    const DenseArgs &a = ma.d;
    if ((int)blockIdx.x >= ma.wl_count[1]) return;
    const uint32_t item = ma.wl_big[blockIdx.x];
    const int gi = (int)(item % (uint32_t)lanes), which = (int)(item / (uint32_t)lanes);
    const int len = a.len[gi];
    if (len == 0) return;
    const int braw = a.bstart[gi];
    const bool sparse_tail = (braw & (1 << 30)) != 0;
    const int bstart = braw & ~(1 << 30);
    const bool live = pos < len && pos <= bstart;
    const bool mine = which == 0 ? (live && pos >= 1) : (live && pos == len - 1 && !sparse_tail);
    if (!mine) return;
    int *cnt = which == 0 ? ma.cntA : ma.cntB;
    const int c = cnt[gi];
    const int g = gi / ma.W, r = gi % ma.W;
    const int mi = which == 0 ? pos : len;
    int n = c < KMAX ? c : KMAX;
    if (c > KMAX) {
        const double *P = (which == 0 ? a.Pa : a.Pb) + (size_t)g * a.N * ma.W + r;
        const double vmax = __longlong_as_double((long long)a.pmax[((size_t)g * (a.Lc + 1) + mi) * ma.W + r]);
        n = block_top_from_column(P, ma.W, a.N, vmax * ma.ratio_lin, vmax, ids, val, ma.force_radix != 0);
    } else {
        const uint32_t *cn = (which == 0 ? ma.candA_node : ma.candB_node) + (size_t)gi * KMAX;
        const double *cv = (which == 0 ? ma.candA_val : ma.candB_val) + (size_t)gi * KMAX;
        for (int j = threadIdx.x; j < n; j += BLOCK) {
            ids[j] = cn[j];
            val[j] = cv[j];
        }
    }
    __syncthreads();
    if (ma.topk > 0 && n < ma.topk && n < a.N && threadIdx.x == 0) {
        const int want = ma.topk < a.N ? ma.topk : a.N;
        const int n0 = n;
        for (uint32_t k = 0; n < want && k < (uint32_t)a.N; k++) {
            bool present = false;
            for (int j = 0; j < n0; j++) present |= ids[j] == k;
            if (!present) {
                ids[n] = k;
                val[n] = 0.0;
                n++;
            }
        }
        cnt[gi] = -n;
    }
    __syncthreads();
    if (cnt[gi] < 0) n = -cnt[gi];
    __syncthreads();
    if (threadIdx.x >= 64) return;
    const uint64_t pidx = ma.lane_pos0[gi] + (uint64_t)(mi - 1);
    if (!emit_mapping<KMAX>(ma.mpool, pidx, ids, val, n, ma.ratio_lin, true, order, ma.topk,
                            (long long)ma.eoff[item])) {
        if (threadIdx.x == 0) atomicOr(&ma.err[gi], SP_ERR_POOL);
    }
    if (threadIdx.x == 0) cnt[gi] = 0;
}

__global__ void __launch_bounds__(BLOCK) gather_logb(const double *logmbB, int Lc, int W, int lanes, double *out) {
    const int gi = blockIdx.x * BLOCK + threadIdx.x;
    if (gi < lanes) out[gi] = logmbB[(size_t)(gi / W) * (Lc + 1) * W + gi % W];
}

__global__ void __launch_bounds__(BLOCK) merge_logp(const uint32_t *lanes, int n, const double *src, double *dst) {
    const int j = blockIdx.x * BLOCK + threadIdx.x;
    if (j < n) dst[lanes[j]] = src[lanes[j]];
}

namespace {
template <int W> void launch_post_collect(const DenseMapArgs &ma, int pos) {
    hipLaunchKernelGGL(post_collect<W>, dim3(ma.d.nblk, ma.d.ng), dim3(BLOCK), 0, current_stream(), ma, pos);
}
void launch_post_collect_w(int W, const DenseMapArgs &ma, int pos) {
    switch (W) {
    case 1: launch_post_collect<1>(ma, pos); break;
    case 2: launch_post_collect<2>(ma, pos); break;
    case 4: launch_post_collect<4>(ma, pos); break;
    case 8: launch_post_collect<8>(ma, pos); break;
    case 16: launch_post_collect<16>(ma, pos); break;
    case 32: launch_post_collect<32>(ma, pos); break;
    case 64: launch_post_collect<64>(ma, pos); break;
    default: PHMM_THROW(PHMM_EINTERNAL, "bad read-group width");
    }
}
}

void mapping_backward_chunk(MapChunk &mc, const std::vector<uint32_t> &sparse_lanes, MappingSink *sink,
                            const Plan &plan, int g0, uint64_t R) {
    hipStream_t s = current_stream();
    CallStats &st = stats();
    phmm_model *m = mc.m;
    const int W = mc.W, lanes = mc.lanes;
    const std::vector<int> &hl = *mc.hl, &hsw = *mc.hsw;
    const std::vector<uint64_t> &lp0 = *mc.lane_pos0;
    const size_t NW = (size_t)m->N * W;

    std::vector<int> hb(lanes, 0);
    std::vector<uint64_t> gp0(lanes + 1, 0);
    int pos_max = -1;
    for (int gi = 0; gi < lanes; gi++) {
        const size_t slot = (size_t)g0 * W + gi;
        if (hl[gi] == 0 || slot >= R) {
            hb[gi] = -1;
            continue;
        }
        gp0[gi] = sink->reads->off[plan.order[slot]];
        if (hsw[gi] < hl[gi]) hb[gi] = hsw[gi] | (1 << 30);
        else hb[gi] = hl[gi] - 1;
        pos_max = std::max(pos_max, hb[gi] & ~(1 << 30));
    }
    DevBuf &ctl = m->wset().aux[3], &pbuf = m->wset().aux[4];
    const bool skip = W == 64 && !knobs().no_bwd_skip && pos_max >= 0;
    const int sseg = seg_size(mc.a.npt);
    const RunSucc *rsucc = skip ? &model_run_successors(m, sseg) : nullptr;
    const size_t sk_nrun = ((size_t)m->N + mc.a.npt - 1) / mc.a.npt;
    size_t cb = 0;
    auto carve = [&](size_t bytes) {
        cb = (cb + 255) / 256 * 256;
        size_t o = cb;
        cb += bytes;
        return o;
    };
    const size_t o_bs = carve(sizeof(int) * lanes), o_ca = carve(sizeof(int) * lanes * 2), o_cb = carve(sizeof(int) * lanes * 2),
                 o_err = carve(sizeof(uint32_t) * lanes), o_cells = carve(sizeof(unsigned long long)), o_lanes = carve(sizeof(uint32_t) * std::max<size_t>(sparse_lanes.size(), 1)),
                 o_lp0 = carve(sizeof(uint64_t) * (lanes + 1)), o_gp0 = carve(sizeof(uint64_t) * (lanes + 1)),
                 o_stop = carve(sizeof(int) * lanes),
                 o_skh = carve(skip ? sizeof(uint32_t) * (size_t)mc.a.ng * rsucc->nseg : 0), o_ska = carve(skip ? 2 * (size_t)mc.a.ng * sk_nrun : 0),
                 o_bn = carve(sizeof(uint32_t) * (size_t)lanes * KMAX * 2), o_bv = carve(sizeof(double) * (size_t)lanes * KMAX * 2),
                 o_an = carve(sizeof(uint32_t) * (size_t)lanes * KMAX * 2), o_av = carve(sizeof(double) * (size_t)lanes * KMAX * 2),
                 o_hand = carve(sizeof(BHandoff) * (size_t)lanes), o_eoff = carve(sizeof(unsigned long long) * 2 * (size_t)lanes),
                 o_wls = carve(sizeof(uint32_t) * 2 * (size_t)lanes), o_wlb = carve(sizeof(uint32_t) * 2 * (size_t)lanes),
                 o_wlc = carve(sizeof(int) * 2), o_lb = carve(sizeof(double) * (size_t)lanes);
    ctl.reserve(cb);
    char *cp = (char *)ctl.p;
    const size_t prun_n = (size_t)mc.ngc * mc.a.nblk8 * BLOCK;
    bool need_pb = false;
    for (int gi = 0; gi < lanes; gi++) need_pb |= hb[gi] >= 0 && !(hb[gi] & (1 << 30));
    pbuf.reserve(((need_pb ? 3 : 2) * (size_t)mc.ngc * NW + prun_n) * sizeof(double));
    unsigned long long top_before = 0;
    HIP_CHECK(hipMemcpyAsync(&top_before, sink->mp.top, sizeof(top_before), hipMemcpyDeviceToHost, s));
    HIP_CHECK(hipStreamSynchronize(s));

    for (int attempt = 0;; attempt++) {
        HIP_CHECK(hipMemsetAsync(cp, 0, o_bn, s));
        HIP_CHECK(hipMemcpyAsync(cp + o_bs, hb.data(), sizeof(int) * lanes, hipMemcpyHostToDevice, s));
        HIP_CHECK(hipMemcpyAsync(cp + o_lp0, lp0.data(), sizeof(uint64_t) * (lanes + 1), hipMemcpyHostToDevice, s));
        HIP_CHECK(hipMemcpyAsync(cp + o_gp0, gp0.data(), sizeof(uint64_t) * (lanes + 1), hipMemcpyHostToDevice, s));
        if (!sparse_lanes.empty())
            HIP_CHECK(hipMemcpyAsync(cp + o_lanes, sparse_lanes.data(), sizeof(uint32_t) * sparse_lanes.size(),
                                     hipMemcpyHostToDevice, s));
        const RecPool mp = sink->mp;

        DenseArgs a = mc.a;
        a.want_freq = 0;
        a.want_map = 1;
        a.bstart = (const int *)(cp + o_bs);
        a.Pa = pbuf.as<double>();
        a.Pb = need_pb ? pbuf.as<double>() + 2 * (size_t)mc.ngc * NW : pbuf.as<double>();
        a.Prun = knobs().no_runmax ? nullptr : pbuf.as<double>() + (need_pb ? 3 : 2) * (size_t)mc.ngc * NW;
        const bool st_on = W == 64 && mc.main_plan;
        if (skip) {
            a.rs_off = rsucc->off.as<uint32_t>();
            a.rs = rsucc->ent.as<uint32_t>();
            a.nseg = (int)rsucc->nseg;
            a.sseg = sseg;
            a.nrun = (int)sk_nrun;
            a.skH = (uint32_t *)(cp + o_skh);
            a.skA = (uint8_t *)(cp + o_ska);
            a.skcells = st_on ? (unsigned long long *)(cp + o_cells) : nullptr;
            HIP_CHECK(hipMemsetAsync(pbuf.p, 0, sizeof(double) * 2 * (size_t)mc.ngc * NW, s));
        }
        HIP_CHECK(hipMemsetAsync(a.cmaxB, 0, sizeof(unsigned long long) * (size_t)a.ng * a.Lc * W, s));
        HIP_CHECK(hipMemsetAsync(a.pmax, 0, sizeof(unsigned long long) * (size_t)a.ng * (a.Lc + 1) * W, s));
        HIP_CHECK(hipMemsetAsync(a.BE, 0, sizeof(int) * (size_t)a.ng * (a.Lc + 1) * W, s));
        HIP_CHECK(hipMemsetAsync(a.Bm, 0, sizeof(double) * (size_t)a.ng * a.bcols * NW, s));
        HIP_CHECK(hipMemsetAsync(a.Bi, 0, sizeof(double) * (size_t)a.ng * a.bcols * NW, s));

        if (!sparse_lanes.empty()) {
            hipLaunchKernelGGL(merge_logp, dim3((unsigned)((sparse_lanes.size() + BLOCK - 1) / BLOCK)), dim3(BLOCK), 0, s,
                               (const uint32_t *)(cp + o_lanes), (int)sparse_lanes.size(), mc.d_logp_sparse, a.logPf);
            SparseBwdArgs ba{};
            ba.M = mc.fa_M;
            ba.d = a;
            ba.W = W;
            ba.Lb = mc.Lfull;
            ba.sw = mc.d_sw;
            ba.bases = mc.d_bases_full;
            ba.fpool = mc.fpool;
            ba.mpool = mp;
            ba.lane_pos0 = (const uint64_t *)(cp + o_lp0);
            ba.map_pos0 = (const uint64_t *)(cp + o_gp0);
            ba.lanes = (const uint32_t *)(cp + o_lanes);
            ba.ratio_lin = mc.ratio_lin;
            ba.topk = mc.topk;
            ba.err = (uint32_t *)(cp + o_err);
            ba.stop = (int *)(cp + o_stop);
            ba.hand = (BHandoff *)(cp + o_hand);
            std::vector<uint32_t> todo;
            std::vector<int> hstop(lanes);
            std::vector<uint32_t> herr2(lanes);
            const bool lean_ok =
                mc.topk == 0 && m->dev.max_degree <= (uint32_t)ADJ_DEG && !knobs().no_lean;
            const bool wide_ok = lean_ok && !knobs().no_wide_class;
            const int slice = mc.Lfull > 6144 ? 4096 : 0;
            std::vector<uint32_t> cont = sparse_lanes, big, fresh;
            bool first = true, any_err = false;
            int bursts = 0;
            auto launch = [&](int kind, int mode, int steps, const std::vector<uint32_t> &who) {
                HIP_CHECK(hipMemcpyAsync(cp + o_lanes, who.data(), sizeof(uint32_t) * who.size(), hipMemcpyHostToDevice, s));
                ba.mode = mode;
                ba.max_steps = steps;
                if (kind == 0 && lean_ok)
                    hipLaunchKernelGGL(lean_backward_kernel, dim3((unsigned)who.size()), dim3(64), 0, s, ba);
                else if (kind == 0)
                    hipLaunchKernelGGL((sparse_backward_kernel<64>), dim3((unsigned)who.size()), dim3(64), 0, s, ba);
                else if (wide_ok)
                    hipLaunchKernelGGL(wide_backward_kernel, dim3((unsigned)who.size()), dim3(WBK_T), 0, s, ba);
                else
                    hipLaunchKernelGGL((sparse_backward_kernel<KMAX>), dim3((unsigned)who.size()), dim3(64), 0, s, ba);
                HIP_CHECK(hipGetLastError());
                st.launches[3]++;
                HIP_CHECK(hipMemcpyAsync(hstop.data(), ba.stop, sizeof(int) * lanes, hipMemcpyDeviceToHost, s));
                HIP_CHECK(hipMemcpyAsync(herr2.data(), ba.err, sizeof(uint32_t) * lanes, hipMemcpyDeviceToHost, s));
                HIP_CHECK(hipStreamSynchronize(s));
            };
            for (int turn = 0; turn < 100000 && !any_err && (!cont.empty() || !big.empty() || !fresh.empty()); turn++) {
                std::vector<uint32_t> ncont;
                if (!cont.empty()) {
                    launch(0, first ? 0 : 1, lean_ok ? slice : 0, cont);
                    for (uint32_t gi : cont) {
                        if (herr2[gi] & ~SP_STOP_SLICE) any_err = true;
                        else if (hstop[gi] == hsw[gi]) continue;
                        else if (herr2[gi] & SP_STOP_SLICE) ncont.push_back(gi);
                        else if (first && hstop[gi] == hl[gi]) fresh.push_back(gi);
                        else big.push_back(gi);
                    }
                    first = false;
                }
                if (any_err) break;
                const int burst = slice > 0 ? (64 << std::min(bursts, 5)) : 0;
                for (int pass = 0; pass < 2 && !any_err; pass++) {
                    std::vector<uint32_t> &who = pass == 0 ? fresh : big;
                    if (who.empty()) continue;
                    launch(1, pass == 0 ? 0 : 1, burst, who);
                    for (uint32_t gi : who) {
                        if (herr2[gi] & ~SP_STOP_SLICE) any_err = true;
                        else if (hstop[gi] != hsw[gi]) ncont.push_back(gi);
                    }
                    who.clear();
                    bursts++;
                }
                cont.swap(ncont);
            }
            todo = cont;
            todo.insert(todo.end(), big.begin(), big.end());
            todo.insert(todo.end(), fresh.begin(), fresh.end());
            if (!todo.empty()) {
                bool perr = false;
                HIP_CHECK(hipMemcpy(herr2.data(), ba.err, sizeof(uint32_t) * lanes, hipMemcpyDeviceToHost));
                for (uint32_t gi : sparse_lanes) perr |= (herr2[gi] & ~SP_STOP_SLICE) != 0;
                if (!perr) PHMM_THROW(PHMM_EINTERNAL, "sparse backward did not finish");
            }
        }
        trace("  sparse backward");
        DenseMapArgs ma{};
        ma.d = a;
        ma.W = W;
        ma.mpool = mp;
        ma.lane_pos0 = (const uint64_t *)(cp + o_gp0);
        ma.ratio_lin = mc.ratio_lin;
        ma.topk = mc.topk;
        ma.err = (uint32_t *)(cp + o_err);
        ma.eoff = (unsigned long long *)(cp + o_eoff);
        ma.wl_small = (uint32_t *)(cp + o_wls);
        ma.wl_big = (uint32_t *)(cp + o_wlb);
        ma.wl_count = (int *)(cp + o_wlc);
        std::vector<int> live_at((size_t)pos_max + 2, 0);
        for (int gi = 0; gi < lanes; gi++)
            if (hb[gi] >= 0) live_at[(size_t)(hb[gi] & ~(1 << 30))]++;
        for (int p = pos_max - 1; p >= 0; p--) live_at[(size_t)p] += live_at[(size_t)p + 1];
        ma.force_radix = knobs().force_radix ? 1 : 0;
        LaunchTimer lt(timing_enabled() && st_on);
        std::unique_lock<std::mutex> dense_lock;
        if (mc.dense_token) dense_lock = std::unique_lock<std::mutex>(*mc.dense_token);
        const int wi = workset_index();
        if (!m->pool->cstream[wi]) {
            int least = 0, greatest = 0;
            HIP_CHECK(hipDeviceGetStreamPriorityRange(&least, &greatest));
            HIP_CHECK(hipStreamCreateWithPriority(&m->pool->cstream[wi], hipStreamNonBlocking, knobs().emit_high_priority ? greatest : least));
        }
        for (auto &e : m->pool->cevent[wi])
            if (!e) HIP_CHECK(hipEventCreateWithFlags(&e, hipEventDisableTiming));
        hipStream_t s2 = knobs().serial_emit ? s : m->pool->cstream[wi];
        hipEvent_t *ev_col = &m->pool->cevent[wi][0], *ev_emit = &m->pool->cevent[wi][2];
        bool emitted[2] = {false, false};
        for (int pos = pos_max; pos >= 0; pos--) {
            const int par = pos & 1;
            a.Pa = pbuf.as<double>() + (size_t)par * mc.ngc * NW;
            ma.d = a;
            ma.cntA = (int *)(cp + o_ca) + (size_t)par * lanes;
            ma.cntB = (int *)(cp + o_cb) + (size_t)par * lanes;
            ma.candA_node = (uint32_t *)(cp + o_an) + (size_t)par * lanes * KMAX;
            ma.candA_val = (double *)(cp + o_av) + (size_t)par * lanes * KMAX;
            ma.candB_node = (uint32_t *)(cp + o_bn) + (size_t)par * lanes * KMAX;
            ma.candB_val = (double *)(cp + o_bv) + (size_t)par * lanes * KMAX;
            if (emitted[par]) HIP_CHECK(hipStreamWaitEvent(s, ev_emit[par], 0));
            lt.begin();
            launch_bwd_step(W, a, pos);
            lt.end();
            launch_post_collect_w(W, ma, pos);
            HIP_CHECK(hipEventRecord(ev_col[par], s));
            HIP_CHECK(hipStreamWaitEvent(s2, ev_col[par], 0));
            hipLaunchKernelGGL(emit_offsets, dim3(1), dim3(1024), 0, s2, ma, pos, lanes);
            {
                const int ub = std::max(1, live_at[(size_t)pos] * (need_pb ? 2 : 1));
                hipLaunchKernelGGL(emit_dense_small, dim3((unsigned)std::min(1024, (ub + BLOCK / 64 - 1) / (BLOCK / 64))), dim3(BLOCK), 0,
                                   s2, ma, pos, lanes);
                hipLaunchKernelGGL(emit_dense_map, dim3((unsigned)ub), dim3(BLOCK), 0, s2, ma, pos, lanes);
            }
            HIP_CHECK(hipEventRecord(ev_emit[par], s2));
            emitted[par] = true;
            if (st_on) st.launches[1]++;
        }
        for (int par = 0; par < 2; par++)
            if (emitted[par]) HIP_CHECK(hipStreamWaitEvent(s, ev_emit[par], 0));
        HIP_CHECK(hipGetLastError());
        const bool want_lb = mc.logb_out && pos_max >= 0 && lanes > 0;
        if (want_lb) {
            launch_bwd_finish(W, a);
            hipLaunchKernelGGL(gather_logb, dim3((unsigned)((lanes + BLOCK - 1) / BLOCK)), dim3(BLOCK), 0, s, (const double *)a.logmbB,
                               a.Lc, W, lanes, (double *)(cp + o_lb));
            HIP_CHECK(hipGetLastError());
        }
        st.ms[1] += lt.total_ms();
        for (int gi = 0; gi < lanes; gi++)
            if (st_on && !a.skcells && hb[gi] >= 0) st.cells[1] += (uint64_t)((hb[gi] & ~(1 << 30)) + 1) * m->N;
        const size_t err_words = (o_cells + sizeof(unsigned long long) - o_err) / sizeof(uint32_t);
        std::vector<uint32_t> herr(err_words);
        HIP_CHECK(hipMemcpyAsync(herr.data(), cp + o_err, sizeof(uint32_t) * err_words, hipMemcpyDeviceToHost, s));
        if (want_lb) HIP_CHECK(hipMemcpyAsync(mc.logb_out, cp + o_lb, sizeof(double) * lanes, hipMemcpyDeviceToHost, s));
        HIP_CHECK(hipStreamSynchronize(s));
        if (a.skcells) {
            unsigned long long nc = 0;
            memcpy(&nc, herr.data() + (o_cells - o_err) / sizeof(uint32_t), sizeof nc);
            st.cells[1] += nc;
        }
        if (dense_lock.owns_lock()) dense_lock.unlock();
        trace("  dense backward+collect");
        bool pool_full = false;
        for (int gi = 0; gi < lanes; gi++) {
            if (herr[gi] & SP_ERR_POOL) pool_full = true;
            else if (herr[gi] & ~SP_STOP_SLICE) PHMM_THROW(PHMM_EINTERNAL, "mapping backward error " + std::to_string(herr[gi]));
        }
        if (!pool_full) break;
        (void)attempt;
        throw SinkOverflow{};
    }
}

__global__ void __launch_bounds__(BLOCK) map_counts(RecPool mp, uint64_t n_pos, uint64_t *cnt) {
    const uint64_t p = (uint64_t)blockIdx.x * BLOCK + threadIdx.x;
    if (p > n_pos) return;
    uint64_t c = 0;
    if (p < n_pos) {
        const uint64_t o1 = mp.off[p];
        if (o1) c = ((const uint32_t *)(mp.base + (o1 - 8)))[0];
    }
    cnt[p] = c;
}
__global__ void __launch_bounds__(BLOCK) map_compact(RecPool mp, uint64_t n_pos, const uint64_t *pos_off, uint32_t *nodes,
                                                     double *logp) {
    const uint64_t p = (uint64_t)blockIdx.x * BLOCK + threadIdx.x;
    if (p >= n_pos) return;
    const uint64_t o1 = mp.off[p];
    if (!o1) return;
    const uint8_t *rec = mp.base + (o1 - 8);
    const uint32_t n = ((const uint32_t *)rec)[0];
    const uint64_t idb = (uint64_t)((n + 1) & ~1u) * 4;
    const uint32_t *ids = (const uint32_t *)(rec + 8);
    const double *lps = (const double *)(rec + 8 + idb);
    const uint64_t w = pos_off[p];
    if (((const uint32_t *)rec)[1] == 0u) {
        for (uint32_t j = 0; j < n; j++) {
            nodes[w + j] = ids[j];
            logp[w + j] = lps[j];
        }
        return;
    }
    for (uint32_t j = 0; j < n; j++) {
        const double v = lps[j];
        const uint32_t id = ids[j];
        uint32_t rank = 0;
        for (uint32_t q = 0; q < n; q++) {
            const double u = lps[q];
            rank += (u > v) || (u == v && ids[q] < id);
        }
        nodes[w + rank] = id;
        logp[w + rank] = v;
    }
}
__global__ void __launch_bounds__(BLOCK) map_read_max(const uint64_t *read_off, uint64_t R, const uint64_t *pos_off,
                                                      uint32_t *out) {
    const uint64_t r = (uint64_t)blockIdx.x * (BLOCK / 64) + (threadIdx.x >> 6);
    const int lane = threadIdx.x & 63;
    if (r >= R) return;
    uint32_t mx = 0;
    for (uint64_t p = read_off[r] + (uint64_t)lane; p < read_off[r + 1]; p += 64) mx = max(mx, (uint32_t)(pos_off[p + 1] - pos_off[p]));
    mx = wave_umax(mx);
    if (lane == 0) out[r] = mx;
}
__global__ void __launch_bounds__(BLOCK) map_probs(const double *logp, uint64_t n, double *prob) {
    const uint64_t j = (uint64_t)blockIdx.x * BLOCK + threadIdx.x;
    if (j < n) prob[j] = exp(logp[j]);
}
static constexpr int NODE_FREQ_WAVES = 4;
__global__ void __launch_bounds__(64 * NODE_FREQ_WAVES) map_node_freq(const uint32_t *sorted_nodes, const double *sorted_prob,
                                                                        uint64_t n, uint32_t N, double *freq) {
    const uint32_t v = blockIdx.x * NODE_FREQ_WAVES + (threadIdx.x >> 6);
    const int lane = threadIdx.x & 63;
    if (v >= N) return;
    uint64_t lo = 0, hi = n;
    while (lo < hi) {
        const uint64_t mid = (lo + hi) >> 1;
        if (sorted_nodes[mid] < v) lo = mid + 1;
        else hi = mid;
    }
    uint64_t e0 = lo, e1 = n;
    while (e0 < e1) {
        const uint64_t mid = (e0 + e1) >> 1;
        if (sorted_nodes[mid] <= v) e0 = mid + 1;
        else e1 = mid;
    }
    double s = 0.0;
    for (uint64_t j = lo + (uint64_t)lane; j < e0; j += 64) s += sorted_prob[j];
    s = wave_sum(s);
    if (lane == 0) freq[v] = s;
}

static void init_sink(phmm_model *m, const phmm_reads *reads, MappingSink &sink, int topk = 0) {
    hipStream_t s = current_stream();
    const uint64_t n_pos = reads->total;
    sink.reads = reads;
    sink.total_pos = n_pos;
    const uint64_t per_pos = topk > 0 ? 16 + 12 * (uint64_t)topk : 160;
    sink.cap = std::max<uint64_t>(m->wset().aux[5].bytes, n_pos * per_pos + reads->R * 131072 + (1u << 20));
    m->wset().aux[5].reserve(sink.cap);
    m->wset().aux[6].reserve(sizeof(unsigned long long) + sizeof(uint64_t) * (n_pos + 1));
    HIP_CHECK(hipMemsetAsync(m->wset().aux[6].p, 0, sizeof(unsigned long long) + sizeof(uint64_t) * (n_pos + 1), s));
    sink.mp.base = m->wset().aux[5].as<uint8_t>();
    sink.mp.cap = sink.cap;
    sink.mp.top = m->wset().aux[6].as<unsigned long long>();
    sink.mp.off = (uint64_t *)(m->wset().aux[6].as<char>() + 8);

}

static void finish_mappings(phmm_model *m, const phmm_reads *reads, MappingSink &sink, const std::vector<double> &lf,
                            const std::vector<double> &lb, phmm_mappings **out, double *out_node_freq) {
    hipStream_t s = current_stream();
    const uint64_t n_pos = reads->total;
    std::unique_ptr<phmm_mappings> mp(new phmm_mappings());
    mp->R = reads->R;
    mp->total_pos = n_pos;
    mp->read_off = reads->off;
// ... 561 lines not shown
```

dbgphmm_amd/csrc/phmm_internal.h:

```cpp
#pragma once

#include <hip/hip_runtime.h>

#include <cstdint>
#include <cstdio>
#include <memory>
#include <mutex>
#include <string>
#include <vector>

#include "../../include/phmm_amd.h"

namespace phmm {

void set_error(const std::string &msg);
int fail(int code, const std::string &msg);

struct Error {
    int code;
    std::string msg;
};
#define PHMM_THROW(code, msg) throw ::phmm::Error{(code), (msg)}
#define HIP_CHECK(expr)                                                                      \
    do {                                                                                     \
// ... 174 lines not shown
    DevBuf par_edge, chi_edge;
    DevBuf trans_lin;
    DevBuf fadj, badj;
    DevBuf prec;
    DevBuf logib;
    size_t logib_len = 0;
    uint32_t max_degree = 0;
};

struct RunSucc {
    int seg = 0;
    uint32_t nseg = 0;
    DevBuf off, ent;
};

}

struct phmm_model {
    uint32_t N = 0, E = 0;
    phmm_params params{};
    phmm::LinParams lin{};
    std::vector<uint8_t> emission;
    std::vector<double> init_logp, trans_logp;
    std::vector<uint32_t> esrc, edst;
    std::vector<uint32_t> par_off, par_node, par_edge, chi_off, chi_node, chi_edge;
    std::vector<double> logib;
    phmm::ModelDev dev;
    double wf_ub_a = 0.0, wf_ub_b = 0.0;
    std::vector<uint32_t> desc_off, desc_node;
    std::mutex rs_mu;
    std::vector<std::unique_ptr<phmm::RunSucc>> rs_cache;
    phmm::DevicePool *pool = nullptr;
    phmm::WorkSet &wset();
};

struct phmm_reads {
    uint64_t R = 0, total = 0;
    std::vector<uint8_t> bases;
    std::vector<uint64_t> off;
    uint64_t max_len = 0;
    mutable phmm::DevBuf d_bases, d_off;
    mutable bool on_device = false;
    mutable std::vector<uint16_t> warm_hint;
    mutable std::vector<uint32_t> last_flags;
};

struct phmm_mappings {
    uint64_t R = 0, total_pos = 0;
    std::vector<uint64_t> read_off;
    std::vector<uint64_t> pos_off;
    std::vector<uint32_t> nodes;
    std::vector<double> logp;
    std::vector<uint32_t> read_max_list;
    std::vector<double> read_logp;
    std::vector<double> read_logp_backward;
    mutable phmm::DevBuf d_pos_off, d_nodes, d_logp;
    int device = -1;
    mutable bool on_device = false;
    mutable bool host_valid = true;
    uint64_t total_entries = 0;
    bool trusted = false;
};
namespace phmm {
void mappings_materialize_host(const phmm_mappings *mp);
}

struct phmm_likelihood {
    phmm_model *m = nullptr;
    const phmm_reads *reads = nullptr;
    const phmm_mappings *mp = nullptr;
    uint32_t min_cn = 0;
    uint64_t T = 0;
    std::vector<uint32_t> cn;
    phmm::DevBuf d_cn, d_val, d_tat;
    std::vector<uint32_t> seen;
    uint32_t stamp = 0;
    uint32_t G = 0, P = 0;
    std::vector<uint64_t> g_off;
    std::vector<uint32_t> g_nodes;
    std::vector<uint32_t> g_of;
    std::vector<uint32_t> g_cn;
    std::vector<uint32_t> g_emit;
    std::vector<uint32_t> g_seen;
    std::vector<uint32_t> g_at;
    uint32_t g_stamp = 0;
    phmm::DevBuf d_g_off, d_g_nodes, d_g_slot, d_bp_off, d_bp_slot;
};

namespace phmm {

struct CallStats {
    double ms[5] = {0, 0, 0, 0, 0};
    uint64_t launches[5] = {0, 0, 0, 0, 0};
    uint64_t cells[5] = {0, 0, 0, 0, 0};
};
CallStats &stats();
bool timing_enabled();

struct LaunchTimer {
    bool on;
    std::vector<hipEvent_t> ev;
    explicit LaunchTimer(bool on_) : on(on_) {}
    ~LaunchTimer() {
        for (auto e : ev) (void)hipEventDestroy(e);
    }
    void begin() {
        if (!on) return;
        hipEvent_t e;
        HIP_CHECK(hipEventCreate(&e));
        HIP_CHECK(hipEventRecord(e, current_stream()));
        ev.push_back(e);
    }
    void end() { begin(); }
    double total_ms() {
        if (!on || ev.empty()) return 0.0;
        HIP_CHECK(hipEventSynchronize(ev.back()));
        double t = 0.0;
        for (size_t k = 0; k + 1 < ev.size(); k += 2) {
            float ms = 0;
            HIP_CHECK(hipEventElapsedTime(&ms, ev[k], ev[k + 1]));
            t += ms;
        }
        return t;
    }
};

void trace(const char *tag);

struct Knobs {
    bool trace = false;
    bool no_lean = false;
    bool no_wide_class = false;
    bool no_packed = false;
    int packed_cpl = 0;
    bool no_exact_hinted = false;
    bool no_exact_dense = false;
    bool wide_hinted = false;
    bool no_wide_hinted = false;
    int wide_hinted_cpb = 0;
    bool no_side_worker = false;
    bool no_wide_handover = false;
    int workers = 1;
    int warm_cols = 0;
    int chunk_groups = 0;
    bool no_keep_all = false;
    int pipeline_min_groups = 8;
    bool no_runmax = false;
    bool force_radix = false;
    bool serial_emit = false;
    bool emit_high_priority = false;
    bool no_dma = false;
    bool bwd_dma = false;
    bool no_bwd_skip = false;
    int dense_streams = 0;
    int dense_w = 0;
    int dense_npt = 0;
    double mem_fraction = 0.0;
};
const Knobs &knobs();
void refresh_knobs();

void model_build_host(phmm_model *m);
void model_upload(phmm_model *m);
const RunSucc &model_run_successors(phmm_model *m, int seg);

void run_dense(phmm_model *m, const phmm_reads *reads, double *out_lf, double *out_lb,
               double *out_nf);
void full_prob_sparse_backward(phmm_model *m, const phmm_reads *reads, double *out_logp, double *out_total);
void backward_sparse_tables(phmm_model *m, const uint8_t *read, uint64_t len, double *b_m, double *b_i, double *b_d,
                            double *b_scal, uint8_t *is_dense);
void run_sparse(phmm_model *m, const phmm_reads *reads, double *out_lf, double *out_lb, double *out_nf);
void run_dense_edges(phmm_model *m, const phmm_reads *reads, double *out_lf, double *out_ef, double *out_if);
struct RecPool;
void full_prob_reads_hinted(phmm_model *m, const phmm_reads *reads, const phmm_mappings *mp, uint32_t n_cand,
                            const double *init_logp, const double *trans_logp, double *out_logp,
                            double *out_total, const RecPool *pool = nullptr, const uint32_t *copy_nums = nullptr,
                            uint32_t min_copy_num = 0);
void full_prob_reads_copy_num_changes(phmm_model *m, const phmm_reads *reads, const phmm_mappings *mp,
                                      const uint32_t *base_cn, uint32_t min_cn, uint32_t n_cand, const uint64_t *chg_off,
                                      const uint32_t *chg_node, const uint32_t *chg_cn, double *out_logp,
                                      double *out_total, uint64_t *out_n_rescored);
void likelihood_refresh(phmm_likelihood *lk);
void likelihood_score_changes(phmm_likelihood *lk, uint32_t n_cand, const uint64_t *chg_off, const uint32_t *chg_node,
                              const uint32_t *chg_cn, double *out_logp, double *out_total, uint64_t *out_n_rescored,
                              bool by_group = false);
void likelihood_move(phmm_likelihood *lk, uint64_t n_chg, const uint32_t *chg_node, const uint32_t *chg_cn,
                     double *out_total, uint64_t *out_n_rescored, bool by_group = false);
void likelihood_current(const phmm_likelihood *lk, uint32_t *out_cn, double *out_logp, double *out_total);
void upload_reads(const phmm_reads *r);
void upload_mappings(const phmm_mappings *mp);
void mappings_map_nodes(phmm_model *m, const phmm_reads *reads, const phmm_mappings *mp_in, const uint32_t *map_off,
                        const uint32_t *map_nodes, uint32_t n_old, phmm_mappings **out);
void generate_mappings_hinted(phmm_model *m, const phmm_reads *reads, const phmm_mappings *mp_in, int use_max_ratio,
                              phmm_mappings **out, double *out_node_freq);
void run_with_mapping_edges(phmm_model *m, const phmm_reads *reads, const phmm_mappings *mp_in, double *out_lf,
                            double *out_ef, double *out_if);
struct MappingSink;
void full_prob_reads_sparse(phmm_model *m, const phmm_reads *reads, double *out_logp, double *out_total,
                            MappingSink *sink, bool by_ratio = true, double *out_logb = nullptr);
void generate_mappings_sparse(phmm_model *m, const phmm_reads *reads, phmm_mappings **out, double *out_node_freq,
                              bool by_ratio = true);
void ensure_logib(phmm_model *m, size_t len);
void put_doubles(double *dst, const double *src_host, size_t n);
void put_bytes(void *dst, const void *src_host, size_t n);
void dense_tables(phmm_model *m, const uint8_t *read, uint64_t len, double *f_m, double *f_i,
                  double *f_d, double *f_scal, double *b_m, double *b_i, double *b_d,
                  double *b_scal);

}
```

dbgphmm_amd/csrc/sparse_dyn.hip:

```cpp
#include <algorithm>
#include <cmath>
#include <cstdlib>
#include <cstring>

#include "dense_internal.h"
#include <condition_variable>
#include <deque>
#include <exception>
#include <functional>
#include <memory>
#include <mutex>
#include <thread>

#include "frontier_dev.h"
#include "sparse_dyn.h"
#include "sparse_fwd_kernel.h"
#include "wide_fwd_kernel.h"
#include "lean_fwd_kernel.h"

namespace phmm {

struct WarmArgs {
    DenseArgs d;
    int *sw;
// ... 214 lines not shown
            a.cand_tot[(size_t)gi * PHMM_MAX_ACTIVE_NODES + j] = stt[j];
        }
        if (threadIdx.x == 0) a.cand_n[gi] = n;
        return;
    }
    unsigned long long lo = 0ull, hi = (unsigned long long)__double_as_longlong(tmax);
    while (lo < hi) {
        const unsigned long long mid = lo + (hi - lo + 1ull) / 2ull;
        int c = 0;
        for (int j = threadIdx.x; j < n; j += BLOCK) c += (unsigned long long)__double_as_longlong(stt[j]) >= mid;
        c = block_count(c, &cnt);
        if (c >= K) lo = mid;
        else hi = mid - 1ull;
    }
    const unsigned long long T = lo;
    int above = 0;
    for (int j = threadIdx.x; j < n; j += BLOCK) above += (unsigned long long)__double_as_longlong(stt[j]) > T;
    above = block_count(above, &cnt);
    const int need_ties = K - above;
    uint32_t blo = 0u, bhi = (uint32_t)N - 1u;
    while (blo < bhi) {
        const uint32_t mid = blo + (bhi - blo) / 2u;
        int c = 0;
        for (int j = threadIdx.x; j < n; j += BLOCK)
            c += ((unsigned long long)__double_as_longlong(stt[j]) == T && sn[j] <= mid) ? 1 : 0;
        c = block_count(c, &cnt);
        if (c >= need_ties) bhi = mid;
        else blo = mid + 1u;
    }
    __syncthreads();
    if (threadIdx.x == 0) cnt = 0;
    __syncthreads();
    for (int j = threadIdx.x; j < n; j += BLOCK) {
        const unsigned long long b = (unsigned long long)__double_as_longlong(stt[j]);
        if (b > T || (b == T && sn[j] <= blo)) {
            const int s = atomicAdd(&cnt, 1);
            if (s < K) {
                a.cand_node[(size_t)gi * PHMM_MAX_ACTIVE_NODES + s] = sn[j];
                a.cand_tot[(size_t)gi * PHMM_MAX_ACTIVE_NODES + s] = stt[j];
            }
        }
    }
    __syncthreads();
    if (threadIdx.x == 0) a.cand_n[gi] = cnt < K ? cnt : K;
}

void launch_select_top(const Top400Args &ta, unsigned n, hipStream_t s) {
    hipLaunchKernelGGL(select_top400, dim3(n), dim3(BLOCK), 0, s, ta);
    HIP_CHECK(hipGetLastError());
}

namespace {

template <int W> void launch_col_count(const WarmArgs &wa, int col) {
    hipLaunchKernelGGL(col_count<W>, dim3(wa.d.nblk, wa.d.ng), dim3(BLOCK), 0, current_stream(), wa, col);
}
void launch_col_count_w(int W, const WarmArgs &wa, int col) {
    switch (W) {
    case 1: launch_col_count<1>(wa, col); break;
    case 2: launch_col_count<2>(wa, col); break;
    case 4: launch_col_count<4>(wa, col); break;
    case 8: launch_col_count<8>(wa, col); break;
    case 16: launch_col_count<16>(wa, col); break;
    case 32: launch_col_count<32>(wa, col); break;
    case 64: launch_col_count<64>(wa, col); break;
    default: PHMM_THROW(PHMM_EINTERNAL, "bad read-group width");
    }
}

}

void full_prob_reads_sparse(phmm_model *m, const phmm_reads *reads, double *out_logp, double *out_total,
                            MappingSink *sink, bool by_ratio, double *out_logb) {
    stats() = CallStats();
    const uint64_t R = reads->R;
    if (m->dev.max_degree > 8)
        PHMM_THROW(PHMM_EINVAL, "sparse path supports node degree <= 8 (MultiDbg MAX_DEGREE is 5)");
    ensure_logib(m, reads->max_len + 1);
    const phmm_params &prm = m->params;
    std::vector<double> lf(R, 0.0);
    std::vector<double> lb(out_logb ? R : 0, 0.0);
    std::vector<uint16_t> new_hint(R, 0);
    std::vector<uint32_t> new_flags(R, 0);
    upload_reads(reads);

    struct PlanCtx {
        Plan plan;
        int64_t lc_cap;
        bool may_defer;
        DevBuf d_order;
        uint64_t max_len = 0;
    };
    struct Item {
        PlanCtx *pc;
        int g0, ngc, Lc, Lfull;
    };
    std::mutex mu;
    std::mutex dense_token;
    std::condition_variable cv;
    std::deque<Item> queue;
    std::deque<Item> side_queue;
    std::thread side_thread;
    bool side_started = false, main_done = false, single_mode = false;
    CallStats side_stats;
    const bool side_on = !knobs().no_side_worker;
    std::vector<std::unique_ptr<PlanCtx>> plans;
    int active = 0;
    std::exception_ptr first_error;
    int n_workers = knobs().workers;
    int64_t warm_cols = 13 + (int64_t)std::ceil(std::log((double)std::max<uint64_t>(m->N, 201) / 200.0) / std::log(4.0));
    warm_cols = std::max<int64_t>(12, warm_cols);
    if (knobs().warm_cols > 0) warm_cols = std::max(4, knobs().warm_cols);
    const int chunk_groups = knobs().chunk_groups;
    uint64_t min_len = UINT64_MAX;
    for (uint64_t r = 0; r < R; r++) min_len = std::min<uint64_t>(min_len, reads->off[r + 1] - reads->off[r]);
    const int map_planes = sink ? (min_len <= (uint64_t)prm.n_warmup + 2 ? 3 : 2) : 0;
    uint64_t limit_total = 0, limit_side = 0;
    {
        const uint64_t est_fpool = reads->total * 1024 + R * 65536 + (1u << 20), est_meta = reads->total * 40,
                       est_ctl = R * (uint64_t)(PHMM_MAX_ACTIVE_NODES * 12 * 5 + WF_CAP * 12 + 4096) + reads->total,
                       est_sink = sink ? reads->total * 176 + R * 131072 + (1u << 21) : 0,
                       est_sel = (uint64_t)256 * m->N * 12;
        const uint64_t est = (est_fpool + est_meta + est_ctl) * 5 / 4 + est_sink + est_sel;
        uint64_t have = m->pool->ws_out.bytes;
        for (const auto &w : m->pool->wsets) {
            have += w.misc.bytes;
            for (int k = 0; k < 16; k++)
                if (k != 4) have += w.aux[k].bytes;
        }
        const uint64_t total = planned_budget(*m->pool), fixed = std::max(est, have);
        limit_total = total > fixed + ((uint64_t)64 << 20) ? total - fixed : (uint64_t)64 << 20;
        uint64_t n_def = std::max<uint64_t>(8, R / 50);
        if (by_ratio && reads->warm_hint.size() == R) {
            n_def = 8;
            for (uint16_t h : reads->warm_hint) n_def += h >= warm_cols ? 1 : 0;
        }
        const uint64_t per_read = ((uint64_t)(prm.n_warmup + 2) * 24 + 4 * 8 + (uint64_t)map_planes * 8) * m->N;
        uint64_t lanes_def = 1;
        while (lanes_def < std::min<uint64_t>(n_def, 64)) lanes_def <<= 1;
        if (n_def > 64) lanes_def = (n_def + 63) / 64 * 64;
        limit_side = std::min<uint64_t>(limit_total / 8, lanes_def * per_read * 9 / 8);
    }
    const uint64_t limit_main = limit_total - limit_side;

    auto enqueue_plan = [&](std::unique_ptr<PlanCtx> pcu, std::deque<Item> &dst) {
        PlanCtx *pc = pcu.get();
        Plan &plan = pc->plan;
        for (uint32_t rd : plan.order) pc->max_len = std::max<uint64_t>(pc->max_len, reads->off[rd + 1] - reads->off[rd]);
        if (by_ratio && reads->warm_hint.size() == reads->R)
            std::stable_sort(plan.order.begin(), plan.order.end(),
                             [&](uint32_t x, uint32_t y) { return reads->warm_hint[x] > reads->warm_hint[y]; });
        const int W = plan.W;
        const size_t NW = (size_t)m->N * W;
        pc->d_order.upload(plan.order.data(), sizeof(uint32_t) * plan.order.size());
        HIP_CHECK(hipStreamSynchronize(current_stream()));
        int target = chunk_groups;
        if (target == 0) target = n_workers > 1 ? std::max(4, (plan.ng_total + 3 * n_workers - 1) / (3 * n_workers)) : plan.ng_total;
        const uint64_t limit = (&dst == &side_queue) ? limit_side : limit_main / (uint64_t)n_workers;
        int g0 = 0;
        while (g0 < plan.ng_total) {
            int Lc = (int)std::min<int64_t>((int64_t)pc->max_len, std::min<int64_t>(prm.n_warmup + 2, pc->lc_cap));
            if (pc->may_defer && g0 == 0 && n_workers == 1) {
                auto cost = [&](int lc) { return (size_t)lc * NW * 24 + 4 * NW * 8 + (sink ? (size_t)map_planes * NW * 8 + (size_t)plan.nblk8 * BLOCK * 8 : 0); };
                const int lc_full = (int)std::min<int64_t>((int64_t)pc->max_len, prm.n_warmup + 2);
                if ((uint64_t)plan.ng_total * cost(lc_full) <= limit && !knobs().no_keep_all) Lc = lc_full;
                else
                    for (int cut = 0; cut <= 2 && Lc - cut >= 8; cut++)
                        if ((uint64_t)plan.ng_total * cost(Lc - cut) <= limit) {
                            Lc -= cut;
                            break;
                        }
            }
            const size_t per_group = (size_t)Lc * NW * 24 + 4 * NW * 8 + (sink ? (size_t)map_planes * NW * 8 + (size_t)plan.nblk8 * BLOCK * 8 : 0);
            int ngc = (int)std::min<uint64_t>(plan.ng_total - g0, std::max<uint64_t>(1, limit / std::max<size_t>(per_group, 1)));
            ngc = std::min(ngc, std::max(1, target));
            int Lfull = 1;
            for (size_t slot = (size_t)g0 * W; slot < std::min<size_t>(plan.order.size(), (size_t)(g0 + ngc) * W); slot++) {
                const uint32_t rd = plan.order[slot];
                Lfull = std::max(Lfull, (int)(reads->off[rd + 1] - reads->off[rd]));
            }
            dst.push_back(Item{pc, g0, ngc, std::min(Lc, Lfull), Lfull});
            g0 += ngc;
        }
        plans.push_back(std::move(pcu));
    };

    std::function<void()> start_side_worker;
    auto run_chunk = [&](const Item &it) {
        hipStream_t s = current_stream();
        CallStats &st = stats();
        DevBuf &warm = m->wset().aux[0];
        DevBuf &fpool = m->wset().aux[1], &fpool_meta = m->wset().aux[2];
        const Plan &plan = it.pc->plan;
        const DevBuf &d_order = it.pc->d_order;
        const int W = plan.W;
        const uint64_t R = plan.order.size();
        const int g0 = it.g0, ngc = it.ngc, Lc = it.Lc, Lfull = it.Lfull;
        std::vector<uint32_t> deferred_ids;
        std::vector<uint32_t> *deferred = it.pc->may_defer ? &deferred_ids : nullptr;
        DenseArgs base{};
        fill_model_args(base, m);
        base.nblk = plan.nblk;
        base.nblk8 = plan.nblk8;
        base.npt = plan.npt;
        base.eall = 0;
        base.want_freq = 0;
        {
        DenseArgs a = base;
        a.ng = ngc;
        a.Lc = Lc;
        size_t tb = 0, mb = 0;
        layout(a, W, false, nullptr, nullptr, tb, mb);
        m->wset().tables.reserve(tb);
        m->wset().misc.reserve(mb);
        layout(a, W, false, m->wset().tables.p, m->wset().misc.p, tb, mb);
        HIP_CHECK(hipMemsetAsync(m->wset().misc.p, 0, mb, s));
        const int lanes = ngc * W;
        size_t wb = 0;
        auto carve = [&](size_t bytes) {
            wb = (wb + 255) / 256 * 256;
            size_t o = wb;
            wb += bytes;
            return o;
        };
        const size_t o_sw = carve(sizeof(int) * lanes), o_cnt = carve(sizeof(int) * lanes),
                     o_cn = carve(sizeof(int) * lanes), o_und = carve(sizeof(int) * 2),
                     o_amb = carve(sizeof(int) * lanes), o_wsub = carve(sizeof(int) * lanes),
                     o_wcnt = carve(sizeof(int) * lanes), o_mode = carve((size_t)lanes),
                     o_cnode = carve(sizeof(uint32_t) * (size_t)lanes * PHMM_MAX_ACTIVE_NODES),
                     o_ctot = carve(sizeof(double) * (size_t)lanes * PHMM_MAX_ACTIVE_NODES),
                     o_lanes = carve(sizeof(uint32_t) * lanes), o_out = carve(sizeof(double) * lanes),
                     o_err = carve(sizeof(uint32_t) * lanes),
                     o_wnode = carve(sizeof(uint32_t) * (size_t)lanes * WF_CAP),
                     o_wtot = carve(sizeof(double) * (size_t)lanes * WF_CAP),
                     o_bases = carve((size_t)ngc * Lfull * W);
        warm.reserve(wb);
        char *wp = (char *)warm.p;
        HIP_CHECK(hipMemsetAsync(wp, 0, o_cnode, s));
        HIP_CHECK(hipMemsetAsync(wp + o_sw, 0xff, sizeof(int) * lanes, s));

        trace("chunk setup");
        if (knobs().trace)
            std::fprintf(stderr, "      chunk: groups %d..%d of %d, W %d, kept columns %d, longest read %d\n", g0, g0 + ngc, plan.ng_total, W, Lc, Lfull);
        std::vector<int> hl((size_t)lanes, 0);
        uint64_t dense_cells = 0;
        for (int gi = 0; gi < lanes; gi++) {
            const size_t slot = (size_t)g0 * W + gi;
            if (slot >= R) continue;
            const uint32_t rd = plan.order[slot];
            hl[gi] = (int)(reads->off[rd + 1] - reads->off[rd]);
        }
        std::vector<double> hib;
        host_logib(m, (size_t)Lc, hib);
        std::vector<int> hlc(hl);
        for (auto &v : hlc) v = std::min(v, Lc);
        {
            StageArgs sa{};
            sa.bases = reads->d_bases.as<uint8_t>();
            sa.off = reads->d_off.as<uint64_t>();
            sa.order = d_order.as<uint32_t>() + (size_t)g0 * W;
            sa.n_slots = (uint32_t)(R - std::min<uint64_t>(R, (uint64_t)g0 * W));
            sa.W = W;
            sa.Lc = Lc;
            sa.Lfull = Lfull;
            sa.out_dense = (uint8_t *)a.bases;
            sa.out_full = (uint8_t *)(wp + o_bases);
            const unsigned per_group = (unsigned)Lfull * W;
            hipLaunchKernelGGL(stage_bases, dim3((per_group + BLOCK - 1) / BLOCK, ngc), dim3(BLOCK), 0, s, sa);
            HIP_CHECK(hipGetLastError());
        }
        HIP_CHECK(hipMemcpyAsync((void *)a.len, hlc.data(), hlc.size() * sizeof(int), hipMemcpyHostToDevice, s));
        HIP_CHECK(hipMemcpyAsync((void *)a.logib, hib.data(), hib.size() * sizeof(double), hipMemcpyHostToDevice, s));
        HIP_CHECK(hipStreamSynchronize(s));

        WarmArgs wa{};
        wa.d = a;
        wa.sw = (int *)(wp + o_sw);
        wa.cnt = (int *)(wp + o_cnt);
        wa.cand_n = (int *)(wp + o_cn);
        wa.undecided = (int *)(wp + o_und);
        wa.n_amb = wa.undecided + 1;
        wa.amb = (int *)(wp + o_amb);
        a.wf_sw = by_ratio ? wa.sw : nullptr;
        a.wf_mode = (const uint8_t *)(wp + o_mode);
        a.wf_sub = (int *)(wp + o_wsub);
        a.wf_cnt = (int *)(wp + o_wcnt);
        a.wf_node = (uint32_t *)(wp + o_wnode);
        a.wf_tot = (double *)(wp + o_wtot);
        a.wf_ratio = std::exp(-prm.active_node_max_ratio);
        a.wf_ub_a = m->wf_ub_a;
        a.wf_ub_b = m->wf_ub_b;
        wa.d = a;
        wa.cand_node = (uint32_t *)(wp + o_cnode);
        wa.cand_tot = (double *)(wp + o_ctot);
        wa.ratio_lin = std::exp(-prm.active_node_max_ratio);
        wa.n_warmup = (int)prm.n_warmup;
        wa.threshold = (int)prm.warmup_threshold;

        trace("staging+upload");
        int pos = 0;
        const bool st_on = W == 64 && (it.pc->may_defer || !by_ratio);
        LaunchTimer lt(timing_enabled() && st_on);
        std::unique_lock<std::mutex> dense_lock(dense_token, std::defer_lock);
        const bool use_token = it.pc->may_defer || !by_ratio;
        if (use_token) dense_lock.lock();
        if (!by_ratio) {
            const int last = std::min<int>((int)prm.n_warmup, Lc);
            for (pos = 0; pos <= last; pos++) {
                lt.begin();
                launch_fwd_step(W, a, pos);
                lt.end();
                if (st_on) st.launches[0]++;
            }
            std::vector<int> fsw(lanes);
            for (int gi = 0; gi < lanes; gi++) fsw[gi] = std::min<int>((int)prm.n_warmup, hl[gi]);
            HIP_CHECK(hipMemcpyAsync(wa.sw, fsw.data(), sizeof(int) * lanes, hipMemcpyHostToDevice, s));
            HIP_CHECK(hipStreamSynchronize(s));
        }
        for (; by_ratio; pos++) {
            lt.begin();
            launch_fwd_step(W, a, pos);
            lt.end();
            if (st_on) st.launches[0]++;
            HIP_CHECK(hipMemsetAsync(wa.undecided, 0, sizeof(int) * 2, s));
            hipLaunchKernelGGL(warm_decide_fused, dim3((lanes + BLOCK / 64 - 1) / (BLOCK / 64)), dim3(BLOCK), 0, s, wa, pos,
                               lanes, W);
// ... 409 lines not shown
```

Measured before the change: 30.13 million.

## Replace dense backward step grid with compacted worklist of active runs

Splits the dense backward step into a marking kernel that computes per-run activity masks and compacts the active runs into a global worklist. A persistent walk kernel then processes only the listed runs. A list-aware post-collect pass and per-run partial sums (rowpart) replace the per-block partials. The goal is to avoid launching and scheduling idle blocks for inactive runs when the skip masks are sparse. In exchange it adds an extra kernel launch per position, atomics for the list and the max reductions, and extra memory for the worklist and row partials.

```diff
diff --git a/dbgphmm_amd/csrc/api.cpp b/dbgphmm_amd/csrc/api.cpp
--- a/dbgphmm_amd/csrc/api.cpp
+++ b/dbgphmm_amd/csrc/api.cpp
@@ -79,6 +79,8 @@
     k.no_runmax = flag("PHMM_NO_RUNMAX");
     k.force_radix = flag("PHMM_FORCE_RADIX");
     k.no_bwd_skip = flag("PHMM_NO_BWD_SKIP");
+    k.no_bwd_worklist = flag("PHMM_NO_BWD_WORKLIST");
+    k.bwd_walk_blocks = std::max(0, num("PHMM_BWD_WALK_BLOCKS", 0));
     k.serial_emit = flag("PHMM_SERIAL_EMIT");
     k.emit_high_priority = flag("PHMM_EMIT_HIGH_PRIORITY");
     k.no_dma = flag("PHMM_NO_DMA");
diff --git a/dbgphmm_amd/csrc/dense.hip b/dbgphmm_amd/csrc/dense.hip
--- a/dbgphmm_amd/csrc/dense.hip
+++ b/dbgphmm_amd/csrc/dense.hip
@@ -1,3 +1,4 @@
+#include <atomic>
 #include <algorithm>
 #include <cmath>
 #include <cstring>
@@ -405,14 +406,45 @@
     return hi + log1p(exp(lo - hi));
 }
 
-template <int W>
+__device__ __forceinline__ void bwd_rowfold(const DenseArgs &a, const int g, const int p, const int r, const int row, double &s1,
+                                            double &s2) {
+    constexpr int W = 64, ROWS = BLOCK / W, U = 4;
+    const double2 *rp = (const double2 *)a.rowpart + ((size_t)(p & 1) * a.ng + g) * a.nrun * W;
+    const uint8_t *am = a.skA + ((size_t)(p & 1) * a.ng + g) * a.nrun;
+    for (int b0 = row; b0 < a.nblk; b0 += ROWS * U) {
+        double2 v[U][ROWS];
+#pragma unroll
+        for (int u = 0; u < U; u++)
+#pragma unroll
+            for (int k = 0; k < ROWS; k++) {
+                const int rho = (b0 + u * ROWS) * ROWS + k;
+                v[u][k] = make_double2(0.0, 0.0);
+                if (rho < a.nrun && am[rho] != 0) v[u][k] = rp[(size_t)rho * W + r];
+            }
+#pragma unroll
+        for (int u = 0; u < U; u++) {
+            double b1 = v[u][0].x, b2 = v[u][0].y;
+#pragma unroll
+            for (int k = 1; k < ROWS; k++) {
+                b1 += v[u][k].x;
+                b2 += v[u][k].y;
+            }
+            s1 += b1;
+            s2 += b2;
+        }
+    }
+}
+
+template <int W, bool LIST = false>
 __device__ __forceinline__ void bwd_chain(const DenseArgs &a, int g, int p, double *lds) {
     constexpr int ROWS = BLOCK / W;
     const int r = threadIdx.x % W, row = threadIdx.x / W;
     const int len = a.len[g * W + r];
     const bool live = p < len && (!a.bstart || p <= (a.bstart[g * W + r] & ~(1 << 30)));
     double s1 = 0.0, s2 = 0.0;
-    if (live) {
+    if (LIST) {
+        if (live) bwd_rowfold(a, g, p, r, row, s1, s2);
+    } else if (live) {
         const double *bp = a.bpart + ((size_t)(p & 1) * a.ng + g) * a.nblk8 * W * 2;
         for (int b = row; b < a.nblk; b += ROWS) {
             s1 += bp[((size_t)b * W + r) * 2 + 0];
@@ -433,66 +465,17 @@
 
 static constexpr int BDMA_DEPTH = 3;
 static constexpr int BDMA_SLOT = 5 * 64;
-template <int W, bool DMA>
-__global__ void __launch_bounds__(BLOCK, (W == 64 ? 4 : PHMM_SMALLW_WAVES)) bwd_step(const DenseArgs a, const int pos) {
-    __shared__ double lds[(BLOCK / 64) * 64];
-    constexpr bool DMA_ = DMA && W == 64;
-    __shared__ double ring[DMA_ ? (BLOCK / 64) * BDMA_DEPTH * BDMA_SLOT : 1];
-    const int g = blockIdx.y + a.g_off;
-    const int lb = xcd_block(blockIdx.x, a.nblk8);
-    constexpr int ROWS = BLOCK / W;
-    const int r = threadIdx.x % W;
-    const int row = threadIdx.x / W;
-    const int len = a.len[g * W + r];
-    const int braw = a.bstart ? a.bstart[g * W + r] : len - 1;
-    const bool sparse_tail = (braw & (1 << 30)) != 0;
-    const int bstart = braw & ~(1 << 30);
-    const bool live = pos < len && pos <= bstart;
-    const bool first = live && pos == len - 1;
+
+struct BwdRowOut {
+    int Epos;
+    double vmax, s1, s2, pmx, pmx2;
+};
+template <int W, bool DMA_>
+__device__ __forceinline__ BwdRowOut bwd_row(const DenseArgs &a, const int pos, const int g, const int r,
+                                             const bool live, const bool first, const bool sparse_tail, const bool walk,
+                                             const int krun, const int hull_first, const int hull_top, double *ring) {
     const LinParams &lp = a.lp;
     const size_t NW = (size_t)a.N * W;
-
-    if (lb == 0 && pos + 1 < a.Lc) bwd_chain<W>(a, g, pos + 1, lds);
-
-    bool compute = true;
-    int hull_first = 0, hull_top = a.npt - 1;
-    if (W == 64 && a.skA) {
-        compute = false;
-        const int rho = __builtin_amdgcn_readfirstlane(lb * ROWS + row);
-        if (__any(live) && rho < a.nrun) {
-            const size_t gs = (size_t)g * a.nseg, gr = (size_t)g * a.nrun, par = (size_t)a.ng * a.nrun;
-            const uint32_t *hh = a.skH + gs;
-            const uint8_t *an = a.skA + (size_t)((pos + 1) & 1) * par + gr;
-            const int sh = pos + 1 < 31 ? pos + 1 : 31;
-            const int sprs = segs_per_run_log2(a.npt), spr = 1 << sprs;
-            const unsigned anyfirst = __any(first) ? 1u : 0u;
-            const int ls = threadIdx.x & 63;
-            const int sg = rho * spr + ls;
-            unsigned f = 0;
-            if (ls < spr && sg < a.nseg) {
-                f = (hh[sg] >> sh) | (((unsigned)an[rho] >> ls) & 1u) | anyfirst;
-                const uint32_t o0 = a.rs_off[sg], o1 = a.rs_off[sg + 1];
-                for (uint32_t q = o0; q < o1 && !f; q++) {
-                    const uint32_t t = a.rs[q];
-                    f = (hh[t] >> sh) | (((unsigned)an[t >> sprs] >> (t & (uint32_t)(spr - 1))) & 1u);
-                }
-            }
-            const unsigned mask = (unsigned)__builtin_amdgcn_readfirstlane((int)(unsigned)__ballot(f != 0));
-            const int kb = rho * a.npt;
-            compute = seg_hull(mask, a.sseg, a.npt - 1 < a.N - 1 - kb ? a.npt - 1 : a.N - 1 - kb, &hull_first, &hull_top);
-            if (ls == 0) a.skA[(size_t)(pos & 1) * par + gr + rho] = (uint8_t)mask;
-        }
-    }
-    if (!__syncthreads_or(live && (compute || lb == 0))) {
-        if (threadIdx.x < W && lb < a.nblk) {
-            double *bp = a.bpart + ((size_t)(pos & 1) * a.ng + g) * a.nblk8 * W * 2;
-            bp[((size_t)lb * W + r) * 2 + 0] = 0.0;
-            bp[((size_t)lb * W + r) * 2 + 1] = 0.0;
-        }
-        if (a.want_map && a.Prun) a.Prun[((size_t)g * a.nblk8 + lb) * BLOCK + threadIdx.x] = 0.0;
-        return;
-    }
-
     int Epos = 0;
     double sc = 1.0;
     if (live && !first) {
@@ -536,9 +519,9 @@
     double vmax = 0.0, s1 = 0.0, s2 = 0.0, pmx = 0.0, pmx2 = 0.0;
     double *Pa = a.want_map ? a.Pa + (size_t)g * NW : nullptr;
     double *Pb = a.want_map ? a.Pb + (size_t)g * NW : nullptr;
-    if (lb < a.nblk && compute) {
+    if (walk) {
         constexpr int H = CHAIN_HOPS;
-        const int kbase = lb * (a.npt * ROWS) + row * a.npt + hull_first;
+        const int kbase = krun + hull_first;
         double E1 = 0.0, E2 = 0.0, E3 = 0.0, E4 = 0.0, E5 = 0.0, Q1 = 0.0, Q2 = 0.0, Q3 = 0.0, Q4 = 0.0, Q5 = 0.0, TE = 0.0;
         int nvalid = 0;
         constexpr int PFB = DMA_ ? BDMA_DEPTH : PHMM_BWD_PF;
@@ -758,6 +741,76 @@
           }
         }
     }
+    return BwdRowOut{Epos, vmax, s1, s2, pmx, pmx2};
+}
+
+__device__ __forceinline__ bool bwd_seg_marked(const DenseArgs &a, const int g, const int pos, const int rho, const int ls,
+                                               const unsigned anyfirst) {
+    const uint32_t *hh = a.skH + (size_t)g * a.nseg;
+    const uint8_t *an = a.skA + ((size_t)((pos + 1) & 1) * a.ng + g) * a.nrun;
+    const int sh = pos + 1 < 31 ? pos + 1 : 31;
+    const int sprs = segs_per_run_log2(a.npt), spr = 1 << sprs;
+    const int sg = rho * spr + ls;
+    unsigned f = (hh[sg] >> sh) | (((unsigned)an[rho] >> ls) & 1u) | anyfirst;
+    const uint32_t o0 = a.rs_off[sg], o1 = a.rs_off[sg + 1];
+    for (uint32_t q = o0; q < o1 && !f; q++) {
+        const uint32_t t = a.rs[q];
+        f = (hh[t] >> sh) | (((unsigned)an[t >> sprs] >> (t & (uint32_t)(spr - 1))) & 1u);
+    }
+    return f != 0;
+}
+__device__ __forceinline__ unsigned bwd_run_mask(const DenseArgs &a, const int g, const int pos, const int rho, const bool first) {
+    const unsigned anyfirst = __any(first) ? 1u : 0u;
+    const int ls = threadIdx.x & 63, spr = 1 << segs_per_run_log2(a.npt);
+    const bool f = ls < spr && rho * spr + ls < a.nseg && bwd_seg_marked(a, g, pos, rho, ls, anyfirst);
+    return (unsigned)__builtin_amdgcn_readfirstlane((int)(unsigned)__ballot(f));
+}
+
+template <int W, bool DMA>
+__global__ void __launch_bounds__(BLOCK, (W == 64 ? 4 : PHMM_SMALLW_WAVES)) bwd_step(const DenseArgs a, const int pos) {
+    __shared__ double lds[(BLOCK / 64) * 64];
+    constexpr bool DMA_ = DMA && W == 64;
+    __shared__ double ring[DMA_ ? (BLOCK / 64) * BDMA_DEPTH * BDMA_SLOT : 1];
+    const int g = blockIdx.y + a.g_off;
+    const int lb = xcd_block(blockIdx.x, a.nblk8);
+    constexpr int ROWS = BLOCK / W;
+    const int r = threadIdx.x % W;
+    const int row = threadIdx.x / W;
+    const int len = a.len[g * W + r];
+    const int braw = a.bstart ? a.bstart[g * W + r] : len - 1;
+    const bool sparse_tail = (braw & (1 << 30)) != 0;
+    const int bstart = braw & ~(1 << 30);
+    const bool live = pos < len && pos <= bstart;
+    const bool first = live && pos == len - 1;
+
+    if (lb == 0 && pos + 1 < a.Lc) bwd_chain<W>(a, g, pos + 1, lds);
+
+    bool compute = true;
+    int hull_first = 0, hull_top = a.npt - 1;
+    if (W == 64 && a.skA) {
+        compute = false;
+        const int rho = __builtin_amdgcn_readfirstlane(lb * ROWS + row);
+        if (__any(live) && rho < a.nrun) {
+            const unsigned mask = bwd_run_mask(a, g, pos, rho, first);
+            const int kb = rho * a.npt;
+            compute = seg_hull(mask, a.sseg, a.npt - 1 < a.N - 1 - kb ? a.npt - 1 : a.N - 1 - kb, &hull_first, &hull_top);
+            if ((threadIdx.x & 63) == 0) a.skA[((size_t)(pos & 1) * a.ng + g) * a.nrun + rho] = (uint8_t)mask;
+        }
+    }
+    if (!__syncthreads_or(live && (compute || lb == 0))) {
+        if (threadIdx.x < W && lb < a.nblk) {
+            double *bp = a.bpart + ((size_t)(pos & 1) * a.ng + g) * a.nblk8 * W * 2;
+            bp[((size_t)lb * W + r) * 2 + 0] = 0.0;
+            bp[((size_t)lb * W + r) * 2 + 1] = 0.0;
+        }
+        if (a.want_map && a.Prun) a.Prun[((size_t)g * a.nblk8 + lb) * BLOCK + threadIdx.x] = 0.0;
+        return;
+    }
+
+    const BwdRowOut o = bwd_row<W, DMA_>(a, pos, g, r, live, first, sparse_tail, lb < a.nblk && compute,
+                                         lb * (a.npt * ROWS) + row * a.npt, hull_first, hull_top, ring);
+    const int Epos = o.Epos;
+    const double vmax = o.vmax, s1 = o.s1, s2 = o.s2, pmx = o.pmx, pmx2 = o.pmx2;
     if (DMA_) asm volatile("s_waitcnt vmcnt(0)" ::: "memory");
     const double bmx = block_reduce_rows<W>(vmax, OpMax(), lds);
     if (threadIdx.x < W && live && lb < a.nblk)
@@ -781,10 +834,95 @@
     if (lb == 0 && threadIdx.x < W && live) a.BE[((size_t)g * (a.Lc + 1) + pos) * W + r] = Epos;
 }
 
-template <int W>
+static constexpr int MARK_ROWS = 256;
+__global__ void __launch_bounds__(BLOCK) bwd_mark(const DenseArgs a, const int pos) {
+    constexpr int W = 64;
+    __shared__ BwdWork ent[MARK_ROWS];
+    __shared__ int s_n, s_base;
+    const int g = blockIdx.y;
+    const int r = threadIdx.x & 63, row = threadIdx.x >> 6;
+    const int len = a.len[g * W + r];
+    const int braw = a.bstart ? a.bstart[g * W + r] : len - 1;
+    const int bstart = braw & ~(1 << 30);
+    const bool live = pos < len && pos <= bstart;
+    const bool first = live && pos == len - 1;
+    if (blockIdx.x == 0) {
+        if (row == 0 && live) {
+            int Epos = 0;
+            if (!first)
+                Epos = a.BE[((size_t)g * (a.Lc + 1) + (pos + 1)) * W + r] + exp_of_bits(a.cmaxB[((size_t)g * a.Lc + (pos + 1)) * W + r]);
+            a.BE[((size_t)g * (a.Lc + 1) + pos) * W + r] = Epos;
+        }
+    }
+    if (!__any(live)) return;
+    const unsigned anyfirst = __any(first) ? 1u : 0u;
+    if (threadIdx.x == 0) s_n = 0;
+    __syncthreads();
+    const int sprs = segs_per_run_log2(a.npt), spr = 1 << sprs;
+    const int rho0 = (int)blockIdx.x * MARK_ROWS;
+    const int rho1 = rho0 + MARK_ROWS < a.nrun ? rho0 + MARK_ROWS : a.nrun;
+    const int ls = threadIdx.x & (spr - 1);
+    for (int base = rho0; base < rho1; base += BLOCK >> sprs) {
+        const int rho = base + ((int)threadIdx.x >> sprs);
+        const bool f = rho < rho1 && rho * spr + ls < a.nseg && bwd_seg_marked(a, g, pos, rho, ls, anyfirst);
+        const unsigned mask = (unsigned)(__ballot(f) >> ((r >> sprs) << sprs)) & ((1u << spr) - 1u);
+        if (ls == 0 && rho < rho1) {
+            const int kb = rho * a.npt;
+            int hull_first = 0, hull_top = 0;
+            const bool compute = seg_hull(mask, a.sseg, a.npt - 1 < a.N - 1 - kb ? a.npt - 1 : a.N - 1 - kb, &hull_first, &hull_top);
+            a.skA[((size_t)(pos & 1) * a.ng + g) * a.nrun + rho] = (uint8_t)mask;
+            if (compute)
+                ent[atomicAdd(&s_n, 1)] = BwdWork{(uint32_t)g * (uint32_t)a.nrun + (uint32_t)rho, (uint32_t)hull_first | ((uint32_t)hull_top << 16)};
+        }
+    }
+    __syncthreads();
+    const int n = s_n;
+    if (threadIdx.x == 0 && n > 0) s_base = atomicAdd(&a.wl_cnt[pos], n);
+    __syncthreads();
+    for (int j = threadIdx.x; j < n; j += BLOCK) a.wl[s_base + j] = ent[j];
+}
+
+template <bool DMA>
+__global__ void __launch_bounds__(BLOCK, 4) bwd_walk(const DenseArgs a, const int pos) {
+    constexpr int W = 64, ROWS = BLOCK / W;
+    __shared__ double ring[DMA ? ROWS * BDMA_DEPTH * BDMA_SLOT : 1];
+    __shared__ double lds[ROWS * 64];
+    if ((int)blockIdx.x < a.ng) {
+        if (pos + 1 < a.Lc) bwd_chain<W, true>(a, (int)blockIdx.x, pos + 1, lds);
+        return;
+    }
+    const int r = threadIdx.x & 63;
+    const int n = a.wl_cnt[pos];
+    const int nw = ((int)gridDim.x - a.ng) * ROWS;
+    for (int i = ((int)blockIdx.x - a.ng) * ROWS + (threadIdx.x >> 6); i < n; i += nw) {
+        const BwdWork w = a.wl[i];
+        const int g = __builtin_amdgcn_readfirstlane((int)(w.row / (uint32_t)a.nrun));
+        const int rho = __builtin_amdgcn_readfirstlane((int)(w.row % (uint32_t)a.nrun));
+        const int hull_first = __builtin_amdgcn_readfirstlane((int)(w.hull & 0xffffu));
+        const int hull_top = __builtin_amdgcn_readfirstlane((int)(w.hull >> 16));
+        const int len = a.len[g * W + r];
+        const int braw = a.bstart ? a.bstart[g * W + r] : len - 1;
+        const bool sparse_tail = (braw & (1 << 30)) != 0;
+        const int bstart = braw & ~(1 << 30);
+        const bool live = pos < len && pos <= bstart;
+        const bool first = live && pos == len - 1;
+        const BwdRowOut o = bwd_row<W, DMA>(a, pos, g, r, live, first, sparse_tail, true, rho * a.npt, hull_first, hull_top, ring);
+        if (DMA) asm volatile("s_waitcnt vmcnt(0)" ::: "memory");
+        if (live && o.vmax > 0.0)
+            atomicMax(&a.cmaxB[((size_t)g * a.Lc + pos) * W + r], (unsigned long long)__double_as_longlong(o.vmax));
+        if (a.Prun) a.Prun[((size_t)g * a.nblk8 + rho / ROWS) * BLOCK + (rho % ROWS) * W + r] = o.pmx;
+        if (live && o.pmx > 0.0)
+            atomicMax(&a.pmax[((size_t)g * (a.Lc + 1) + pos) * W + r], (unsigned long long)__double_as_longlong(o.pmx));
+        if (first && !sparse_tail && o.pmx2 > 0.0)
+            atomicMax(&a.pmax[((size_t)g * (a.Lc + 1) + len) * W + r], (unsigned long long)__double_as_longlong(o.pmx2));
+        ((double2 *)a.rowpart)[(((size_t)(pos & 1) * a.ng + g) * a.nrun + rho) * W + r] = make_double2(o.s1, o.s2);
+    }
+}
+
+template <int W, bool LIST = false>
 __global__ void __launch_bounds__(BLOCK) bwd_finish(const DenseArgs a) {
     __shared__ double lds[(BLOCK / 64) * 64];
-    bwd_chain<W>(a, blockIdx.x, 0, lds);
+    bwd_chain<W, LIST>(a, blockIdx.x, 0, lds);
 }
 
 __global__ void __launch_bounds__(BLOCK) freq_reduce(const double *accg, int ng, int N, double *out, int accumulate) {
@@ -1016,8 +1154,37 @@
     PHMM_W_SWITCH(W, CALL_)
 #undef CALL_
 }
+template <bool DMA> static int walk_blocks() {
+    static std::atomic<int> nb[64] = {};
+    int dev = 0;
+    HIP_CHECK(hipGetDevice(&dev));
+    const int slot = dev >= 0 && dev < 64 ? dev : 0;
+    int v = dev == slot ? nb[slot].load(std::memory_order_relaxed) : 0;
+    if (v == 0) {
+        int cus = 0, per = 0;
+        HIP_CHECK(hipDeviceGetAttribute(&cus, hipDeviceAttributeMultiprocessorCount, dev));
+        HIP_CHECK(hipOccupancyMaxActiveBlocksPerMultiprocessor(&per, bwd_walk<DMA>, BLOCK, 0));
+        v = 4 * std::max(1, cus) * std::max(1, per);
+        if (dev == slot) nb[slot].store(v, std::memory_order_relaxed);
+    }
+    return v;
+}
+int bwd_worklist_blocks() {
+    const int nb = knobs().bwd_dma ? walk_blocks<true>() : walk_blocks<false>(), cap = knobs().bwd_walk_blocks;
+    return cap > 0 ? cap : nb;
+}
+void launch_bwd_worklist(const DenseArgs &a, int pos) {
+    hipStream_t s = current_stream();
+    if (!a.want_map || a.g_off != 0 || !a.skA || !a.wl || !a.wl_cnt || !a.rowpart || a.npt > 0xffff || (uint64_t)a.ng * (uint64_t)a.nrun > 0xffffffffull)
+        PHMM_THROW(PHMM_EINTERNAL, "bad arguments of the list form of the dense backward step");
+    hipLaunchKernelGGL(bwd_mark, dim3((unsigned)((a.nrun + MARK_ROWS - 1) / MARK_ROWS), (unsigned)a.ng), dim3(BLOCK), 0, s, a, pos);
+    const dim3 grid((unsigned)(bwd_worklist_blocks() + a.ng));
+    if (knobs().bwd_dma) hipLaunchKernelGGL(bwd_walk<true>, grid, dim3(BLOCK), 0, s, a, pos);
+    else hipLaunchKernelGGL(bwd_walk<false>, grid, dim3(BLOCK), 0, s, a, pos);
+}
 template <int W> static void launch_bwd_fin(const DenseArgs &a) {
-    hipLaunchKernelGGL(bwd_finish<W>, dim3(a.ng), dim3(BLOCK), 0, current_stream(), a);
+    if (W == 64 && a.rowpart) hipLaunchKernelGGL((bwd_finish<64, true>), dim3(a.ng), dim3(BLOCK), 0, current_stream(), a);
+    else hipLaunchKernelGGL(bwd_finish<W>, dim3(a.ng), dim3(BLOCK), 0, current_stream(), a);
 }
 void launch_bwd_finish(int W, const DenseArgs &a) {
 #define CALL_(w) launch_bwd_fin<w>(a)
diff --git a/dbgphmm_amd/csrc/dense_internal.h b/dbgphmm_amd/csrc/dense_internal.h
--- a/dbgphmm_amd/csrc/dense_internal.h
+++ b/dbgphmm_amd/csrc/dense_internal.h
@@ -9,6 +9,10 @@
 
 static constexpr double LN2 = 0.693147180559945309417232121458;
 static constexpr int BLOCK = 256;
+
+struct BwdWork {
+    uint32_t row, hull;
+};
 
 struct DenseArgs {
     int N, ng, Lc, nblk, npt;
@@ -62,6 +66,9 @@
     uint8_t *skA = nullptr;
     int nrun = 0, nseg = 0, sseg = 1;
     unsigned long long *skcells = nullptr;
+    BwdWork *wl = nullptr;
+    int *wl_cnt = nullptr;
+    double *rowpart = nullptr;
 };
 static constexpr int WF_CAP = 1024;
 
@@ -80,6 +87,8 @@
 void launch_fwd_step(int W, const DenseArgs &a, int pos);
 void launch_fwd_finish(int W, const DenseArgs &a);
 void launch_bwd_step(int W, const DenseArgs &a, int pos);
+void launch_bwd_worklist(const DenseArgs &a, int pos);
+int bwd_worklist_blocks();
 void launch_bwd_finish(int W, const DenseArgs &a);
 
 struct ExactTables {
diff --git a/dbgphmm_amd/csrc/mapping_flow.hip b/dbgphmm_amd/csrc/mapping_flow.hip
--- a/dbgphmm_amd/csrc/mapping_flow.hip
+++ b/dbgphmm_amd/csrc/mapping_flow.hip
@@ -496,6 +496,53 @@
     }
 }
 
+__global__ void __launch_bounds__(BLOCK) post_collect_list(const DenseMapArgs ma, const int pos) {
+    const DenseArgs &a = ma.d;
+    constexpr int W = 64, ROWS = BLOCK / W;
+    const int r = threadIdx.x & 63;
+    const int n = a.wl_cnt[pos];
+    const int nw = (int)gridDim.x * ROWS;
+    const size_t NW = (size_t)a.N * W;
+    for (int i = (int)blockIdx.x * ROWS + (threadIdx.x >> 6); i < n; i += nw) {
+        const uint32_t wr = a.wl[i].row;
+        const int g = (int)(wr / (uint32_t)a.nrun), rho = (int)(wr % (uint32_t)a.nrun);
+        const int gi = g * W + r;
+        const int len = a.len[gi];
+        const int braw = a.bstart[gi];
+        const bool sparse_tail = (braw & (1 << 30)) != 0;
+        const int bstart = braw & ~(1 << 30);
+        const bool live = pos < len && pos <= bstart;
+        const int k0 = rho * a.npt;
+        for (int which = 0; which < 2; which++) {
+            if (!(which == 0 ? live && pos >= 1 : live && pos == len - 1 && !sparse_tail)) continue;
+            const double *P = (which == 0 ? a.Pa : a.Pb) + (size_t)g * NW;
+            const int mi = which == 0 ? pos : len;
+            const double thr = __longlong_as_double((long long)a.pmax[((size_t)g * (a.Lc + 1) + mi) * W + r]) * ma.ratio_lin;
+            if (which == 0 && a.Prun) {
+                const double rm = a.Prun[((size_t)g * a.nblk8 + rho / ROWS) * BLOCK + (rho % ROWS) * W + r];
+                if (!(rm > 0.0 && rm > thr)) continue;
+            }
+            int local = 0;
+            for (int j = 0; j < a.npt && k0 + j < a.N; j++) {
+                const double t = P[(size_t)(k0 + j) * W + r];
+                local += (t > 0.0 && t > thr) ? 1 : 0;
+            }
+            if (local == 0) continue;
+            int slot = atomicAdd(&(which == 0 ? ma.cntA : ma.cntB)[gi], local);
+            uint32_t *cn = (which == 0 ? ma.candA_node : ma.candB_node) + (size_t)gi * KMAX;
+            double *cv = (which == 0 ? ma.candA_val : ma.candB_val) + (size_t)gi * KMAX;
+            for (int j = 0; j < a.npt && k0 + j < a.N && slot < KMAX; j++) {
+                const double t = P[(size_t)(k0 + j) * W + r];
+                if (t > 0.0 && t > thr) {
+                    cn[slot] = (uint32_t)(k0 + j);
+                    cv[slot] = t;
+                    slot++;
+                }
+            }
+        }
+    }
+}
+
 __device__ int block_top_radix(const double *col, int stride, int N, double thr, uint32_t *ids, double *val) {
     __shared__ unsigned int hist[256];
     __shared__ unsigned long long s_prefix;
@@ -911,6 +958,9 @@
     }
     DevBuf &ctl = m->wset().aux[3], &pbuf = m->wset().aux[4];
     const bool skip = W == 64 && !knobs().no_bwd_skip && pos_max >= 0;
+    const size_t walk_waves = (size_t)bwd_worklist_blocks() * (BLOCK / 64);
+    const bool worklist = skip && !knobs().no_bwd_worklist &&
+                          (knobs().bwd_walk_blocks > 0 || (size_t)mc.a.ng * (((size_t)m->N + mc.a.npt - 1) / mc.a.npt) >= walk_waves);
     const int sseg = seg_size(mc.a.npt);
     const RunSucc *rsucc = skip ? &model_run_successors(m, sseg) : nullptr;
     const size_t sk_nrun = ((size_t)m->N + mc.a.npt - 1) / mc.a.npt;
@@ -926,17 +976,20 @@
                  o_lp0 = carve(sizeof(uint64_t) * (lanes + 1)), o_gp0 = carve(sizeof(uint64_t) * (lanes + 1)),
                  o_stop = carve(sizeof(int) * lanes),
                  o_skh = carve(skip ? sizeof(uint32_t) * (size_t)mc.a.ng * rsucc->nseg : 0), o_ska = carve(skip ? 2 * (size_t)mc.a.ng * sk_nrun : 0),
+                 o_wlcnt = carve(worklist ? sizeof(int) * (size_t)mc.a.Lc : 0),
                  o_bn = carve(sizeof(uint32_t) * (size_t)lanes * KMAX * 2), o_bv = carve(sizeof(double) * (size_t)lanes * KMAX * 2),
                  o_an = carve(sizeof(uint32_t) * (size_t)lanes * KMAX * 2), o_av = carve(sizeof(double) * (size_t)lanes * KMAX * 2),
                  o_hand = carve(sizeof(BHandoff) * (size_t)lanes), o_eoff = carve(sizeof(unsigned long long) * 2 * (size_t)lanes),
                  o_wls = carve(sizeof(uint32_t) * 2 * (size_t)lanes), o_wlb = carve(sizeof(uint32_t) * 2 * (size_t)lanes),
-                 o_wlc = carve(sizeof(int) * 2), o_lb = carve(sizeof(double) * (size_t)lanes);
+                 o_wlc = carve(sizeof(int) * 2), o_lb = carve(sizeof(double) * (size_t)lanes),
+                 o_wl = carve(worklist ? sizeof(BwdWork) * (size_t)mc.a.ng * sk_nrun : 0);
     ctl.reserve(cb);
     char *cp = (char *)ctl.p;
     const size_t prun_n = (size_t)mc.ngc * mc.a.nblk8 * BLOCK;
     bool need_pb = false;
     for (int gi = 0; gi < lanes; gi++) need_pb |= hb[gi] >= 0 && !(hb[gi] & (1 << 30));
-    pbuf.reserve(((need_pb ? 3 : 2) * (size_t)mc.ngc * NW + prun_n) * sizeof(double));
+    const size_t rowpart_n = worklist ? 2 * (size_t)mc.ngc * sk_nrun * W * 2 : 0;
+    pbuf.reserve(((need_pb ? 3 : 2) * (size_t)mc.ngc * NW + prun_n + rowpart_n) * sizeof(double));
     unsigned long long top_before = 0;
     HIP_CHECK(hipMemcpyAsync(&top_before, sink->mp.top, sizeof(top_before), hipMemcpyDeviceToHost, s));
     HIP_CHECK(hipStreamSynchronize(s));
@@ -968,6 +1021,11 @@
             a.skH = (uint32_t *)(cp + o_skh);
             a.skA = (uint8_t *)(cp + o_ska);
             a.skcells = st_on ? (unsigned long long *)(cp + o_cells) : nullptr;
+            if (worklist) {
+                a.wl = (BwdWork *)(cp + o_wl);
+                a.wl_cnt = (int *)(cp + o_wlcnt);
+                a.rowpart = pbuf.as<double>() + (need_pb ? 3 : 2) * (size_t)mc.ngc * NW + prun_n;
+            }
             HIP_CHECK(hipMemsetAsync(pbuf.p, 0, sizeof(double) * 2 * (size_t)mc.ngc * NW, s));
         }
         HIP_CHECK(hipMemsetAsync(a.cmaxB, 0, sizeof(unsigned long long) * (size_t)a.ng * a.Lc * W, s));
@@ -1081,6 +1139,10 @@
         for (int p = pos_max - 1; p >= 0; p--) live_at[(size_t)p] += live_at[(size_t)p + 1];
         ma.force_radix = knobs().force_radix ? 1 : 0;
         LaunchTimer lt(timing_enabled() && st_on);
+        const int pcl_blocks = !worklist ? 0
+                               : knobs().bwd_walk_blocks > 0
+                                   ? bwd_worklist_blocks()
+                                   : (int)std::min<size_t>(((size_t)a.ng * sk_nrun + BLOCK / 64 - 1) / (BLOCK / 64), (size_t)4 * bwd_worklist_blocks());
         std::unique_lock<std::mutex> dense_lock;
         if (mc.dense_token) dense_lock = std::unique_lock<std::mutex>(*mc.dense_token);
         const int wi = workset_index();
@@ -1106,9 +1168,12 @@
             ma.candB_val = (double *)(cp + o_bv) + (size_t)par * lanes * KMAX;
             if (emitted[par]) HIP_CHECK(hipStreamWaitEvent(s, ev_emit[par], 0));
             lt.begin();
-            launch_bwd_step(W, a, pos);
+            if (worklist) launch_bwd_worklist(a, pos);
+            else launch_bwd_step(W, a, pos);
             lt.end();
-            launch_post_collect_w(W, ma, pos);
+            if (worklist)
+                hipLaunchKernelGGL(post_collect_list, dim3((unsigned)pcl_blocks), dim3(BLOCK), 0, s, ma, pos);
+            else launch_post_collect_w(W, ma, pos);
             HIP_CHECK(hipEventRecord(ev_col[par], s));
             HIP_CHECK(hipStreamWaitEvent(s2, ev_col[par], 0));
             hipLaunchKernelGGL(emit_offsets, dim3(1), dim3(1024), 0, s2, ma, pos, lanes);
diff --git a/dbgphmm_amd/csrc/phmm_internal.h b/dbgphmm_amd/csrc/phmm_internal.h
--- a/dbgphmm_amd/csrc/phmm_internal.h
+++ b/dbgphmm_amd/csrc/phmm_internal.h
@@ -350,6 +350,8 @@
     bool no_dma = false;
     bool bwd_dma = false;
     bool no_bwd_skip = false;
+    bool no_bwd_worklist = false;
+    int bwd_walk_blocks = 0;
     int dense_streams = 0;
     int dense_w = 0;
     int dense_npt = 0;
diff --git a/dbgphmm_amd/csrc/sparse_dyn.hip b/dbgphmm_amd/csrc/sparse_dyn.hip
--- a/dbgphmm_amd/csrc/sparse_dyn.hip
+++ b/dbgphmm_amd/csrc/sparse_dyn.hip
@@ -390,6 +390,7 @@
                              [&](uint32_t x, uint32_t y) { return reads->warm_hint[x] > reads->warm_hint[y]; });
         const int W = plan.W;
         const size_t NW = (size_t)m->N * W;
+        const size_t rowpart_bytes = W == 64 ? 2 * (((size_t)m->N + plan.npt - 1) / plan.npt) * W * 16 : 0;
         pc->d_order.upload(plan.order.data(), sizeof(uint32_t) * plan.order.size());
         HIP_CHECK(hipStreamSynchronize(current_stream()));
         int target = chunk_groups;
@@ -399,7 +400,7 @@
         while (g0 < plan.ng_total) {
             int Lc = (int)std::min<int64_t>((int64_t)pc->max_len, std::min<int64_t>(prm.n_warmup + 2, pc->lc_cap));
             if (pc->may_defer && g0 == 0 && n_workers == 1) {
-                auto cost = [&](int lc) { return (size_t)lc * NW * 24 + 4 * NW * 8 + (sink ? (size_t)map_planes * NW * 8 + (size_t)plan.nblk8 * BLOCK * 8 : 0); };
+                auto cost = [&](int lc) { return (size_t)lc * NW * 24 + 4 * NW * 8 + (sink ? (size_t)map_planes * NW * 8 + (size_t)plan.nblk8 * BLOCK * 8 + rowpart_bytes : 0); };
                 const int lc_full = (int)std::min<int64_t>((int64_t)pc->max_len, prm.n_warmup + 2);
                 if ((uint64_t)plan.ng_total * cost(lc_full) <= limit && !knobs().no_keep_all) Lc = lc_full;
                 else
@@ -409,7 +410,7 @@
                             break;
                         }
             }
-            const size_t per_group = (size_t)Lc * NW * 24 + 4 * NW * 8 + (sink ? (size_t)map_planes * NW * 8 + (size_t)plan.nblk8 * BLOCK * 8 : 0);
+            const size_t per_group = (size_t)Lc * NW * 24 + 4 * NW * 8 + (sink ? (size_t)map_planes * NW * 8 + (size_t)plan.nblk8 * BLOCK * 8 + rowpart_bytes : 0);
             int ngc = (int)std::min<uint64_t>(plan.ng_total - g0, std::max<uint64_t>(1, limit / std::max<size_t>(per_group, 1)));
             ngc = std::min(ngc, std::max(1, target));
             int Lfull = 1;
```

Result: faster. 30.87 million (median of 6 runs) (+2.5%).
